# weixiaopassking/GS-LIVM

Measured on AMD Instinct MI355X. Metric: rasterizer fwd+bwd Mpixels/s @1920x1080, 2000000 Gaussians (ms_per_step = ms/frame), higher is better.
Workload: dtype f32; 1 GPU; C3: 2000000 Gaussians, 1920x1080, SH degree 0, 1 view per GPU per step, fwd+bwd + Adam step; view_threads=1, camera=one fixed view, near_entries=0, parallelism=view-parallel x1, adam_in_step=True, optimizer=one-kernel tail: activation chain rule + Adam + next activations (HIP), loss=seeded

## Files before the change

gs-livm_amd/__init__.py:

```python
from . import multiview, synthetic
from ._capi import (GsrError, LIB_PATH, NumRendered, emit_guard_trips, last_num_rendered, lib, mailbox_slow_path_last, mark_visible,
                    set_binning_capacity_hint, speculation_stats, set_near_far, set_near_far_thread, set_reference_rects_thread, async_outcomes_pending, set_near_far_hints, last_near_far, set_far_speculation, last_far_skipped, profile_enable, profile_read,
                    pose_gradient, rasterize_backward, rasterize_forward, reference_rects, set_reference_rects, state_views)
from .loss import (DeltaDepthLoss, ExposureLoss, LidarDepthLoss, PhotometricLoss, SimilarityLoss, delta_depth_loss, delta_pose,
                   apply_exposure, exposure_photometric_loss, identity_exposure, lidar_depth_image, lidar_depth_loss,
                   photometric_loss, raster_K, reference_window_1d, similarity_loss,
                   world_to_camera)
from .covis import (KeyframeVisibility, covisibility, iou, observation_count, overlap_coefficient,
                    visibility_pack, visibility_remap)
from .metrics import depth_to_u8, evaluate_keyframes, image_metrics, psnr, side_by_side, to_u8
from .model import FusedActivations, FusedAdam, GaussianParameters, GrowableAdam, GrowableGaussians, VoxelIndex, prune_rows
from . import ply
from .rasterizer import (GaussianRasterizationSettings, GaussianRasterizer,
                         rasterize_gaussians)
from .render_utils import Camera, get_projection_matrix, render, render_full, se3_exp



def torch_ops():
    import importlib.util
    import os
    import torch
    lib()
    path = os.path.join(os.path.dirname(os.path.abspath(__file__)), "_gsraster_torch.so")
    if not os.path.exists(path):
        raise RuntimeError("_gsraster_torch.so not built: run `python gs-livm_amd/build.py`")
    spec = importlib.util.spec_from_file_location("_gsraster_torch", path)
    mod = importlib.util.module_from_spec(spec)
    spec.loader.exec_module(mod)
    return mod


__all__ = ["KeyframeVisibility", "visibility_pack", "covisibility", "observation_count", "visibility_remap", "iou", "overlap_coefficient", "ExposureLoss", "exposure_photometric_loss", "apply_exposure", "identity_exposure", "LidarDepthLoss", "lidar_depth_image", "lidar_depth_loss", "raster_K", "world_to_camera", "prune_rows", "image_metrics", "psnr", "to_u8", "side_by_side", "depth_to_u8", "evaluate_keyframes", "DeltaDepthLoss", "delta_depth_loss", "delta_pose", "SimilarityLoss", "similarity_loss", "VoxelIndex", "PhotometricLoss", "photometric_loss", "reference_window_1d", "FusedActivations", "FusedAdam", "GaussianParameters", "GrowableAdam", "GrowableGaussians", "ply", "GaussianRasterizationSettings", "GaussianRasterizer", "rasterize_gaussians", "Camera", "render", "render_full", "se3_exp", "pose_gradient", "get_projection_matrix", "rasterize_forward",
           "rasterize_backward", "mark_visible", "state_views", "set_reference_rects", "reference_rects", "last_num_rendered", "set_binning_capacity_hint", "speculation_stats", "emit_guard_trips", "mailbox_slow_path_last", "set_near_far", "set_near_far_thread", "set_reference_rects_thread", "async_outcomes_pending", "set_near_far_hints", "last_near_far", "set_far_speculation", "last_far_skipped", "NumRendered", "lib", "torch_ops", "synthetic", "multiview", "GsrError", "LIB_PATH"]
```

gs-livm_amd/_capi.py:

```python
import ctypes as C
import os

import torch

_HERE = os.path.dirname(os.path.abspath(__file__))
LIB_PATH = os.environ.get("GSR_LIB", os.path.join(_HERE, "libgsraster_hip.so"))

ALLOC_FN = C.CFUNCTYPE(C.c_void_p, C.c_void_p, C.c_size_t)


class GeometryView(C.Structure):
    _fields_ = [(n, C.c_void_p) for n in
                ("depths", "radii", "splats", "cov3D", "tiles_touched", "point_offsets", "clamped", "depth_order",
                 "num_rendered", "gpack")]


class BinningView(C.Structure):
    _fields_ = [("point_list", C.c_void_p)]


class ImageView(C.Structure):
    _fields_ = [(n, C.c_void_p) for n in ("ranges", "final_T", "n_contrib", "quad_last", "ranges_far")]


class MailboxEvent(C.Structure):
    _fields_ = [("count", C.c_uint), ("ticket_expected", C.c_uint32), ("ticket_seen_before_query", C.c_uint32),
                ("elapsed_us", C.c_double), ("ticket_seen_after_query", C.c_uint32), ("first_query_result", C.c_int),
                ("visible_at_query", C.c_int), ("queries", C.c_uint), ("longest_query_us", C.c_double),
                ("longest_poll_gap_us", C.c_double)]


class NumRendered(int):

    def __new__(cls, exact, key):
        obj = super().__new__(cls, exact)
        obj.key = int(key)
        return obj


def _key(R):
    return int(getattr(R, "key", R))


_lib = None

EXPORTS = ("gsr_forward", "gsr_backward", "gsr_backward_depth", "gsr_mark_visible", "gsr_geometry_bytes", "gsr_image_bytes",
           "gsr_binning_bytes", "gsr_geometry_view_of", "gsr_binning_view_of", "gsr_image_view_of",
           "gsr_higher_msb", "gsr_last_error", "gsr_abi_version", "gsr_kernel_count", "gsr_kernel_name",
           "gsr_profile_enable", "gsr_profile_enable_only", "gsr_profile_read", "gsr_mailbox_slow_path_hits", "gsr_activate", "gsr_activate_backward", "gsr_adam_step",
           "gsr_photometric_loss", "gsr_photometric_loss_workspace", "gsr_init_gaussians", "gsr_ply_row_floats",
           "gsr_pack_ply_rows", "gsr_model_step", "gsr_set_reference_rects", "gsr_reference_rects",
           "gsr_last_num_rendered", "gsr_set_binning_capacity_hint", "gsr_speculative_forwards",
           "gsr_speculation_overflows", "gsr_emit_guard_trips", "gsr_mailbox_slow_path_last", "gsr_set_near_far", "gsr_near_far",
           "gsr_last_near_far", "gsr_set_near_far_hints", "gsr_near_far_forwards", "gsr_set_far_speculation",
           "gsr_last_far_skipped", "gsr_far_skips", "gsr_far_skip_misses", "gsr_async_far_frames",
           "gsr_near_budget_scale", "gsr_near_budget_feedback", "gsr_near_far_pause", "gsr_set_near_far_thread",
           "gsr_set_reference_rects_thread", "gsr_async_outcomes_pending", "gsr_async_outcomes_lost",
           "gsr_frame_note_misses", "gsr_similarity_loss", "gsr_similarity_loss_workspace",
           "gsr_delta_depth_loss", "gsr_delta_depth_loss_workspace", "gsr_image_metrics",
           "gsr_image_metrics_workspace", "gsr_pack_image_u8", "gsr_pack_depth_u8", "gsr_prune_workspace",
           "gsr_prune_mark", "gsr_prune_compact", "gsr_lidar_depth_image", "gsr_lidar_depth_loss",
           "gsr_lidar_depth_loss_workspace", "gsr_density_accumulate", "gsr_densify_workspace", "gsr_densify_mark",
           "gsr_densify_apply", "gsr_pose_gradient", "gsr_pose_gradient_workspace", "gsr_exposure_loss",
           "gsr_exposure_loss_workspace", "gsr_apply_exposure", "gsr_visibility_words", "gsr_visibility_pack",
           "gsr_covisibility", "gsr_observation_count", "gsr_visibility_remap")


def lib():
    global _lib
    if _lib is not None:
        return _lib
    if not os.path.exists(LIB_PATH):
        raise RuntimeError(
            "libgsraster_hip.so not built: run `python gs-livm_amd/build.py` (needs hipcc). "
            "gs_livm_amd has no CPU fallback.")
    L = C.CDLL(LIB_PATH)
    vp, ci, cf, sz = C.c_void_p, C.c_int, C.c_float, C.c_size_t
    L.gsr_forward.restype = ci
    L.gsr_forward.argtypes = [ALLOC_FN, vp, ALLOC_FN, vp, ALLOC_FN, vp, ci, ci, ci, vp, ci, ci, vp, vp, vp, vp, vp, cf,
                              vp, vp, vp, vp, vp, cf, cf, ci, vp, vp, vp, vp, ci, vp]
    L.gsr_backward.restype = ci
    L.gsr_backward.argtypes = [ci, ci, ci, ci, vp, ci, ci, vp, vp, vp, vp, cf, vp, vp, vp, vp, vp, cf, cf, vp, vp, vp,
                               vp, vp, vp, vp, vp, vp, vp, vp, vp, vp, vp, vp, ci, vp]
    L.gsr_backward_depth.restype = ci
    L.gsr_backward_depth.argtypes = L.gsr_backward.argtypes[:25] + [vp] + L.gsr_backward.argtypes[25:34] + [vp, ci, vp]
    L.gsr_mark_visible.restype = ci
    L.gsr_mark_visible.argtypes = [ci, vp, vp, vp, vp, vp]
    L.gsr_pose_gradient_workspace.restype = sz
    L.gsr_pose_gradient_workspace.argtypes = [ci]
    L.gsr_pose_gradient.restype = ci
    L.gsr_pose_gradient.argtypes = [ci, ci, ci, vp, vp, cf, vp, vp, vp, vp, cf, cf, vp, vp, vp, vp, vp, vp, vp, sz, vp]
    for n in ("gsr_geometry_bytes", "gsr_binning_bytes"):
        getattr(L, n).restype = sz
        getattr(L, n).argtypes = [ci]
    L.gsr_image_bytes.restype = sz
    L.gsr_image_bytes.argtypes = [ci, ci]
    L.gsr_geometry_view_of.argtypes = [vp, ci, C.POINTER(GeometryView)]
    L.gsr_binning_view_of.argtypes = [vp, ci, C.POINTER(BinningView)]
    L.gsr_image_view_of.argtypes = [vp, ci, ci, C.POINTER(ImageView)]
    L.gsr_higher_msb.restype = C.c_uint32
    L.gsr_higher_msb.argtypes = [C.c_uint32]
    L.gsr_last_error.restype = C.c_char_p
    L.gsr_abi_version.restype = ci
    L.gsr_kernel_count.restype = ci
    L.gsr_kernel_name.restype = C.c_char_p
    L.gsr_kernel_name.argtypes = [ci]
    L.gsr_profile_enable.argtypes = [ci]
    L.gsr_profile_enable_only.argtypes = [C.POINTER(ci), ci]
    L.gsr_set_reference_rects.restype = ci
    L.gsr_set_reference_rects.argtypes = [ci]
    L.gsr_reference_rects.restype = ci
    L.gsr_reference_rects.argtypes = []
    L.gsr_last_num_rendered.restype = ci
    L.gsr_last_num_rendered.argtypes = []
    L.gsr_set_binning_capacity_hint.restype = C.c_longlong
    L.gsr_set_binning_capacity_hint.argtypes = [C.c_longlong]
    for n in ("gsr_speculative_forwards", "gsr_speculation_overflows", "gsr_emit_guard_trips"):
        getattr(L, n).restype = C.c_ulonglong
        getattr(L, n).argtypes = []
    L.gsr_set_near_far.restype = ci
    L.gsr_set_near_far.argtypes = [ci]
    L.gsr_near_far.restype = ci
    L.gsr_near_far.argtypes = []
    L.gsr_last_near_far.restype = ci
    L.gsr_last_near_far.argtypes = [C.POINTER(C.c_uint), C.POINTER(C.c_uint)]
    L.gsr_set_near_far_hints.restype = None
    L.gsr_set_near_far_hints.argtypes = [C.c_longlong, C.c_longlong]
    L.gsr_near_far_forwards.restype = C.c_ulonglong
    L.gsr_near_far_forwards.argtypes = []
    L.gsr_set_far_speculation.restype = ci
    L.gsr_set_far_speculation.argtypes = [ci]
    L.gsr_last_far_skipped.restype = ci
    L.gsr_last_far_skipped.argtypes = []
    L.gsr_near_budget_scale.restype = C.c_uint
    L.gsr_near_budget_scale.argtypes = []
    L.gsr_near_budget_feedback.restype = C.c_uint
    L.gsr_near_budget_feedback.argtypes = [C.c_uint, C.c_uint, C.c_uint]
    L.gsr_near_far_pause.restype = ci
    L.gsr_near_far_pause.argtypes = [ci]
    for n in ("gsr_far_skips", "gsr_far_skip_misses", "gsr_async_far_frames", "gsr_async_outcomes_lost",
              "gsr_frame_note_misses", "gsr_similarity_loss", "gsr_similarity_loss_workspace"):
        getattr(L, n).restype = C.c_ulonglong
        getattr(L, n).argtypes = []
    for n in ("gsr_set_near_far_thread", "gsr_set_reference_rects_thread"):
        getattr(L, n).restype = ci
        getattr(L, n).argtypes = [ci]
    L.gsr_async_outcomes_pending.restype = ci
    L.gsr_async_outcomes_pending.argtypes = []
    L.gsr_mailbox_slow_path_last.restype = ci
    L.gsr_mailbox_slow_path_last.argtypes = [C.POINTER(MailboxEvent)]
    L.gsr_mailbox_slow_path_hits.restype = C.c_ulonglong
    L.gsr_mailbox_slow_path_hits.argtypes = []
    L.gsr_profile_read.restype = ci
    L.gsr_profile_read.argtypes = [ci, C.POINTER(C.c_double), C.POINTER(ci)]
    L.gsr_activate.restype = ci
    L.gsr_activate.argtypes = [ci, ci] + [vp] * 9 + [vp]
    L.gsr_activate_backward.restype = ci
    L.gsr_activate_backward.argtypes = [ci, ci] + [vp] * 12 + [vp]
    L.gsr_photometric_loss_workspace.restype = sz
    L.gsr_photometric_loss_workspace.argtypes = [ci, ci, ci]
    L.gsr_photometric_loss.restype = ci
    L.gsr_photometric_loss.argtypes = [ci, ci, ci, vp, vp, C.POINTER(cf), cf, vp, vp, vp, sz, vp]
    L.gsr_exposure_loss_workspace.restype = sz
    L.gsr_exposure_loss_workspace.argtypes = [ci, ci, ci]
    L.gsr_exposure_loss.restype = ci
    L.gsr_exposure_loss.argtypes = [ci, ci, ci, vp, vp, vp, C.POINTER(cf), cf, vp, vp, vp, vp, sz, vp]
    L.gsr_apply_exposure.restype = ci
    L.gsr_apply_exposure.argtypes = [ci, ci, ci, vp, vp, vp, vp]
    L.gsr_similarity_loss_workspace.restype = sz
    L.gsr_similarity_loss_workspace.argtypes = [ci, ci]
    L.gsr_similarity_loss.restype = ci
    L.gsr_similarity_loss.argtypes = [ci, ci, ci, vp, vp, vp, vp, cf, vp, vp, vp, ci, vp, sz, vp]
    L.gsr_delta_depth_loss_workspace.restype = sz
    L.gsr_delta_depth_loss_workspace.argtypes = [ci, ci]
    L.gsr_delta_depth_loss.restype = ci
    L.gsr_delta_depth_loss.argtypes = [ci, ci, vp, vp, vp, vp, C.POINTER(cf), C.POINTER(cf), C.POINTER(cf), cf, vp, vp,
                                       vp, vp, vp, sz, vp]
    L.gsr_lidar_depth_image.restype = ci
    L.gsr_lidar_depth_image.argtypes = [ci, vp, C.POINTER(cf), C.POINTER(cf), ci, ci, cf, cf, vp, vp, vp]
    L.gsr_lidar_depth_loss_workspace.restype = sz
    L.gsr_lidar_depth_loss_workspace.argtypes = [ci, ci]
    L.gsr_lidar_depth_loss.restype = ci
    L.gsr_lidar_depth_loss.argtypes = [ci, ci, vp, vp, vp, cf, cf, vp, vp, vp, vp, sz, vp]
    L.gsr_image_metrics_workspace.restype = sz
    L.gsr_image_metrics_workspace.argtypes = [ci, ci, ci]
    L.gsr_image_metrics.restype = ci
    L.gsr_image_metrics.argtypes = [ci, ci, ci, vp, vp, C.POINTER(cf), vp, vp, vp, sz, vp]
    L.gsr_pack_image_u8.restype = ci
    L.gsr_pack_image_u8.argtypes = [ci, ci, vp, ci, vp, sz, vp]
    L.gsr_pack_depth_u8.restype = ci
    L.gsr_pack_depth_u8.argtypes = [ci, ci, vp, cf, vp, sz, vp]
    L.gsr_prune_workspace.restype = sz
    L.gsr_prune_workspace.argtypes = [ci]
    L.gsr_prune_mark.restype = ci
    L.gsr_prune_mark.argtypes = [ci, vp, vp, vp, vp, vp, cf, cf, ci, vp, vp, vp, vp, sz, vp]
    L.gsr_prune_compact.restype = ci
    L.gsr_prune_compact.argtypes = [ci, ci, C.POINTER(vp), C.POINTER(vp), C.POINTER(ci), vp, vp, vp]
    L.gsr_density_accumulate.restype = ci
    L.gsr_density_accumulate.argtypes = [ci, vp, vp, vp, vp]
    L.gsr_densify_workspace.restype = sz
    L.gsr_densify_workspace.argtypes = [ci]
    L.gsr_densify_mark.restype = ci
    L.gsr_densify_mark.argtypes = [ci, vp, vp, cf, cf, ci, vp, vp, vp, vp, sz, vp]
    L.gsr_densify_apply.restype = ci
    L.gsr_densify_apply.argtypes = [ci, ci, ci, vp, vp, C.c_ulonglong] + [vp] * 6 + [C.POINTER(vp), C.POINTER(vp), vp, vp]
    ll = C.c_longlong
    L.gsr_visibility_words.restype = sz
    L.gsr_visibility_words.argtypes = [ci]
    L.gsr_visibility_pack.restype = ci
    L.gsr_visibility_pack.argtypes = [ci, vp, vp, vp, ci, vp]
    L.gsr_covisibility.restype = ci
    L.gsr_covisibility.argtypes = [ci, vp, ll, ci, vp, ll, ci, vp, vp, vp, vp]
    L.gsr_observation_count.restype = ci
    L.gsr_observation_count.argtypes = [ci, vp, ll, ci, ci, ci, vp, vp, vp]
    L.gsr_visibility_remap.restype = ci
    L.gsr_visibility_remap.argtypes = [ci, vp, ll, ci, vp, vp, vp, ll, ci, vp]
    L.gsr_init_gaussians.restype = ci
    L.gsr_init_gaussians.argtypes = [ci, ci, vp, vp, vp, cf] + [vp] * 6 + [vp]
    L.gsr_ply_row_floats.restype = sz
    L.gsr_ply_row_floats.argtypes = [ci]
    L.gsr_pack_ply_rows.restype = ci
    L.gsr_pack_ply_rows.argtypes = [ci, ci] + [vp] * 7 + [vp]
    L.gsr_model_step.restype = ci
    L.gsr_model_step.argtypes = [ci, ci, C.POINTER(vp), C.POINTER(vp), C.POINTER(vp)] + [vp] * 9 + \
        [C.POINTER(cf), C.c_double, C.c_double, C.c_double, ci, vp]
    L.gsr_adam_step.restype = ci
    L.gsr_adam_step.argtypes = [ci, C.POINTER(vp), C.POINTER(vp), C.POINTER(vp), C.POINTER(vp), C.POINTER(sz),
                                C.POINTER(cf), C.c_double, C.c_double, C.c_double, ci, ci, vp]
    _lib = L
    return L

# ... 118 lines not shown
        out = out + (dL_dconic,)
    return out + (dL_ddepths,) if grad_depth is not None else out


def pose_gradient(means3D, radii, scales, rotations, scale_modifier, cov3D_precomp, viewmatrix, projmatrix, tan_fovx,
                  tan_fovy, image_height, image_width, dL_dmeans2D, dL_dconic, dL_dmeans3D, dL_ddepths=None,
                  workspace=None):
    dev = means3D.device
    P = int(means3D.size(0))
    L = lib()
    need = int(L.gsr_pose_gradient_workspace(P))
    if workspace is None:
        workspace = torch.empty(need, dtype=torch.uint8, device=dev)
    out = torch.empty(6, dtype=torch.float32, device=dev)
    rotations = _rot16(rotations)
    _check(L.gsr_pose_gradient(P, int(image_width), int(image_height), _ptr(means3D), _ptr(scales),
                               float(scale_modifier), _ptr(rotations), _ptr(cov3D_precomp), _ptr(viewmatrix),
                               _ptr(projmatrix), float(tan_fovx), float(tan_fovy), _ptr(radii), _ptr(dL_dmeans2D),
                               _ptr(dL_dconic), _ptr(dL_ddepths), _ptr(dL_dmeans3D), _ptr(out), _ptr(workspace),
                               workspace.numel(), _stream()))
    return out


def last_num_rendered():
    return int(lib().gsr_last_num_rendered())


def set_binning_capacity_hint(capacity):
    return int(lib().gsr_set_binning_capacity_hint(-1 if capacity is None else int(capacity)))


def speculation_stats():
    L = lib()
    return dict(speculative_forwards=int(L.gsr_speculative_forwards()), overflows=int(L.gsr_speculation_overflows()),
                near_far_forwards=int(L.gsr_near_far_forwards()), far_skips=int(L.gsr_far_skips()),
                far_skip_misses=int(L.gsr_far_skip_misses()), async_far_frames=int(L.gsr_async_far_frames()),
                async_outcomes_lost=int(L.gsr_async_outcomes_lost()), frame_note_misses=int(L.gsr_frame_note_misses()),
                near_budget_scale_q8=int(L.gsr_near_budget_scale()),
                mailbox_slow_path_hits=int(L.gsr_mailbox_slow_path_hits()))


def emit_guard_trips():
    return int(lib().gsr_emit_guard_trips())


def mailbox_slow_path_last():
    ev = MailboxEvent()
    _check(lib().gsr_mailbox_slow_path_last(C.byref(ev)))
    return {n: getattr(ev, n) for n, _ in MailboxEvent._fields_}


def set_near_far(on):
    return bool(lib().gsr_set_near_far(int(bool(on))))


def set_near_far_thread(mode):
    prev = int(lib().gsr_set_near_far_thread(-1 if mode is None else int(bool(mode))))
    return None if prev < 0 else bool(prev)


def async_outcomes_pending():
    return int(lib().gsr_async_outcomes_pending())


def set_near_far_hints(near_entries_per_tile=None, far_capacity=None):
    lib().gsr_set_near_far_hints(-1 if near_entries_per_tile is None else int(near_entries_per_tile),
                                 -1 if far_capacity is None else int(far_capacity))


def set_far_speculation(mode):
    return int(lib().gsr_set_far_speculation(-1 if mode is None else int(bool(mode))))


def last_far_skipped():
    return bool(lib().gsr_last_far_skipped())


def last_near_far():
    a, b = C.c_uint(0), C.c_uint(0)
    split = bool(lib().gsr_last_near_far(C.byref(a), C.byref(b)))
    return split, int(a.value), int(b.value)


def set_reference_rects(on):
    return bool(lib().gsr_set_reference_rects(int(bool(on))))


def set_reference_rects_thread(mode):
    prev = int(lib().gsr_set_reference_rects_thread(-1 if mode is None else int(bool(mode))))
    return None if prev < 0 else bool(prev)


def reference_rects():
    return bool(lib().gsr_reference_rects())


def mark_visible(means3D, viewmatrix, projmatrix):
    P = int(means3D.size(0))
    present = torch.zeros((P,), dtype=torch.bool, device=means3D.device)
    if P:
        _check(lib().gsr_mark_visible(P, _ptr(means3D), _ptr(viewmatrix), _ptr(projmatrix),
                                      C.c_void_p(present.data_ptr()), _stream()))
    return present


def _sub(blob, ptr, count, dtype):
    if not ptr or count == 0:
        return None
    off = int(ptr) - blob.data_ptr()
    nbytes = count * torch.empty((), dtype=dtype).element_size()
    return blob[off:off + nbytes].view(dtype)


def state_views(geomBuffer, binningBuffer, imageBuffer, P, R, W, H):
    L = lib()
    gv, bv, iv = GeometryView(), BinningView(), ImageView()
    T = ((W + 15) // 16) * ((H + 15) // 16)
    out = {}
    if P:
        _check(L.gsr_geometry_view_of(_ptr(geomBuffer), P, C.byref(gv)))
        splats = _sub(geomBuffer, gv.splats, P * 12, torch.float32).view(P, 12)
        gpack = _sub(geomBuffer, gv.gpack, P * 2, torch.int32).view(P, 2)
        out.update(depths=splats[:, 9],
                   radii=_sub(geomBuffer, gv.radii, P, torch.int32),
                   splats=splats,
                   cov3D=_sub(geomBuffer, gv.cov3D, P * 6, torch.float32).view(P, 6),
                   tiles_touched=gpack[:, 0],
                   point_offsets=_sub(geomBuffer, gv.point_offsets, P, torch.int32),
                   clamped=_sub(geomBuffer, gv.clamped, P, torch.uint8),
                   depth_order=_sub(geomBuffer, gv.depth_order, P, torch.int32))
        _check(L.gsr_image_view_of(_ptr(imageBuffer), W, H, C.byref(iv)))
        out.update(ranges=_sub(imageBuffer, iv.ranges, T * 2, torch.int32).view(T, 2),
                   final_T=_sub(imageBuffer, iv.final_T, W * H, torch.float32).view(H, W),
                   n_contrib=_sub(imageBuffer, iv.n_contrib, W * H, torch.int32).view(H, W),
                   quad_last=_sub(imageBuffer, iv.quad_last, T * 4, torch.int32).view(T, 4))
        counters = _sub(geomBuffer, gv.num_rendered, 16, torch.int32).cpu().tolist()
        split = counters[12] == 1
        exact = counters[6] + counters[8] if split else counters[0]
        out.update(num_rendered=exact, near_far=split, counters=counters)
        key = _key(R)
        if exact:
            _check(L.gsr_binning_view_of(_ptr(binningBuffer), key, C.byref(bv)))
            raw = _sub(binningBuffer, bv.point_list, key, torch.int32)
            ra = out["ranges"].long()
            rb = _sub(imageBuffer, iv.ranges_far, T * 2, torch.int32).view(T, 2).long()
            seg_start = torch.stack([ra[:, 0], rb[:, 0]], 1).reshape(-1)
            seg_len = torch.stack([ra[:, 1] - ra[:, 0], rb[:, 1] - rb[:, 0]], 1).reshape(-1)
            total = int(seg_len.sum())
            excl = torch.cumsum(seg_len, 0) - seg_len
            idx = torch.repeat_interleave(seg_start - excl, seg_len) + torch.arange(total, device=ra.device)
            point_list = raw[idx]
            ln = seg_len.view(T, 2).sum(1)
            ends = torch.cumsum(ln, 0)
            ranges = torch.stack([ends - ln, ends], 1)
            ranges[ln == 0] = 0
            out.update(ranges_near=out["ranges"], ranges_far=rb.int(), ranges=ranges.int())
            tile_ids = torch.repeat_interleave(torch.arange(T, device=ra.device), ln)
            dbits = out["depths"].view(torch.int32)[point_list.long()].long() & 0xFFFFFFFF
            out.update(tile_ids=tile_ids, point_list=point_list, keys=(tile_ids.long() << 32) | dbits)
    return out


def profile_enable(on=True, only=None):
    L = lib()
    if on and only is not None:
        names = [L.gsr_kernel_name(i).decode() for i in range(L.gsr_kernel_count())]
# ... 340 lines not shown
```

gs-livm_amd/csrc/api.hip:

```cpp
#include "../../include/gsraster.h"

#include <algorithm>
#include <atomic>
#include <mutex>
#include <cstdarg>
#include <cstdio>
#include <cstdlib>
#include <cstring>
#include <chrono>
#include <cmath>
#include <unordered_map>
#include <vector>

#include "gsr_api.hpp"
#include "gsr_internal.hpp"

using namespace gsr;

static thread_local char g_err[512] = "";

namespace gsr {
int fail(int code, const char* fmt, ...) {
  va_list ap;
  va_start(ap, fmt);
  vsnprintf(g_err, sizeof(g_err), fmt, ap);
  va_end(ap);
  return code;
}
void clear_error() { g_err[0] = 0; }
}

#define STAGE(expr)                                                                               \
  do {                                                                                            \
    HIP_TRY(expr);                                                                                \
    if (debug) HIP_TRY(hipStreamSynchronize(stream));                                             \
  } while (0)

namespace gsr {
const Env& env() {
  static const Env e = [] {
    const auto set = [](const char* v) { return v != nullptr; };
    const auto not_zero = [](const char* v) { return !(v && v[0] == '0'); };
    Env x;
    const char* v = getenv("GSR_REFERENCE_RECTS");
    x.reference_rects = v && v[0] && v[0] != '0';
    x.near_far = not_zero(getenv("GSR_NEAR_FAR"));
    x.async_far = not_zero(getenv("GSR_ASYNC_FAR"));
    x.sync_forward = set(getenv("GSR_SYNC_FORWARD"));
    v = getenv("GSR_NEAR_ENTRIES");
    x.near_entries = v ? atol(v) : 320;
    v = getenv("GSR_NEAR_FAR_MIN_RATIO_Q2");
    x.near_far_min_ratio_q2 = v ? strtoull(v, nullptr, 10) : 12ull;
    x.full_depth_sort = set(getenv("GSR_FULL_DEPTH_SORT"));
    x.depth_hist_pass = set(getenv("GSR_DEPTH_HIST_PASS"));
    v = getenv("GSR_PRE_HIST_MIN_P");
    x.pre_hist_min_p = v ? std::max(0L, atol(v)) : -1;
    x.ranges_from_keys = set(getenv("GSR_RANGES_FROM_KEYS"));
    x.tile_sort_lsd = set(getenv("GSR_TILE_SORT_LSD"));
    x.sort_two_level_scan = set(getenv("GSR_SORT_TWO_LEVEL_SCAN"));
    x.sort_ballot_rank = set(getenv("GSR_SORT_BALLOT_RANK"));
    x.blend_backward_quads = set(getenv("GSR_BLEND_BACKWARD_QUADS"));
    x.blend_backward_tiles = set(getenv("GSR_BLEND_BACKWARD_TILES"));
    x.bwd_image_order = set(getenv("GSR_BWD_IMAGE_ORDER"));
    x.gbwd_all = set(getenv("GSR_GBWD_ALL"));
    x.host_trace = set(getenv("GSR_HOST_TRACE"));
    return x;
  }();
  return e;
}
}

namespace gsr {
std::atomic<bool> g_prof_on{false};
std::atomic<unsigned long long> g_prof_mask{~0ull};
thread_local bool t_prof_suppress = false;
static std::mutex g_ev_mu;
static std::vector<hipEvent_t> g_ev;
static std::vector<int> g_ev_id;
static size_t g_ev_used = 0;
void prof_begin(int id, hipStream_t s) {
  g_ev_mu.lock();
  if (g_ev_used == g_ev_id.size()) {
    hipEvent_t a, b;
    if (hipEventCreate(&a) != hipSuccess || hipEventCreate(&b) != hipSuccess) {
      g_prof_on = false;
      g_ev_id.push_back(-1);
      g_ev.push_back(nullptr); g_ev.push_back(nullptr);
      return;
    }
    g_ev.push_back(a); g_ev.push_back(b); g_ev_id.push_back(id);
  }
  g_ev_id[g_ev_used] = id;
  if (g_ev[2 * g_ev_used]) (void)hipEventRecord(g_ev[2 * g_ev_used], s);
}
void prof_end(hipStream_t s) {
  if (g_ev_used < g_ev_id.size() && g_ev[2 * g_ev_used + 1]) {
    (void)hipEventRecord(g_ev[2 * g_ev_used + 1], s);
    g_ev_used++;
  }
  g_ev_mu.unlock();
}
}
static const char* const kKernelNames[K_COUNT] = {
    "k_preprocess", "k_point_offsets", "k_scan_offsets", "k_emit",
    "k_sort_hist", "k_sort_scan_chunks", "k_sort_scan_top", "k_sort_scatter", "k_tile_ranges", "k_blend_forward",
    "k_blend_backward", "k_compact_touched", "k_gather_records", "k_gaussian_backward", "k_mark_visible", "k_sort_hist[depth]",
    "k_sort_scan_chunks[depth]", "k_sort_scan_top[depth]", "k_sort_scatter[depth]", "k_activate",
    "k_activate_backward", "k_adam", "k_loss_forward", "k_loss_finalize", "k_loss_backward", "k_init_gaussians", "k_pack_ply_rows", "k_model_step", "k_tile_order", "k_live_sat", "k_compact_near",
    "k_simi_nearest", "k_simi_points", "k_simi_grads",
    "k_delta_project", "k_delta_sample", "k_delta_scatter", "k_delta_convert",
    "k_visibility",
    "k_lidar_clear", "k_lidar_splat", "k_lidar_convert", "k_lidar_loss_forward", "k_lidar_loss_finish",
    "k_lidar_loss_grads",
    "k_density_accumulate", "k_densify_mark", "k_densify_scan", "k_densify_rank", "k_densify_apply",
    "k_pose_partials", "k_pose_finish",
    "k_exposure_loss_forward", "k_exposure_loss_backward", "k_exposure_loss_finish", "k_apply_exposure",
    "k_metrics_forward", "k_metrics_finalize", "k_pack_image_u8", "k_pack_depth_u8",
    "k_prune_mark", "k_prune_scan", "k_prune_rank", "k_prune_compact"};
static_assert(K_COUNT <= 64, "g_prof_mask is one 64-bit word");

extern "C" {

int gsr_kernel_count(void) { return K_COUNT; }
const char* gsr_kernel_name(int id) { return (id >= 0 && id < K_COUNT) ? kKernelNames[id] : ""; }
int gsr_profile_enable(int on) {
  std::lock_guard<std::mutex> lk(g_ev_mu);
  if (on) g_ev_used = 0;
  g_prof_on = on != 0;
  g_prof_mask = ~0ull;
  return GSR_OK;
}
int gsr_profile_enable_only(const int* kernel_ids, int n) {
  if (!kernel_ids && n > 0) return fail(GSR_ERR_INVALID_ARGUMENT, "null kernel id list");
  unsigned long long m = 0;
  for (int i = 0; i < n; i++) {
    if (kernel_ids[i] < 0 || kernel_ids[i] >= K_COUNT) return fail(GSR_ERR_INVALID_ARGUMENT, "bad kernel id");
    m |= 1ull << kernel_ids[i];
  }
  std::lock_guard<std::mutex> lk(g_ev_mu);
  g_ev_used = 0;
  g_prof_mask = m;
  g_prof_on = true;
  return GSR_OK;
}
int gsr_profile_read(int max_ids, double* total_ms, int* launches) {
  const int n = max_ids < K_COUNT ? max_ids : (int)K_COUNT;
  std::lock_guard<std::mutex> lk(g_ev_mu);
// ... 958 lines not shown
  lazy_resolve(g_ctx);
  return (int)g_ctx.last_R;
}
int gsr_set_near_far(int on) { return near_far_flag().exchange(on != 0 ? 1 : 0); }
int gsr_set_near_far_thread(int mode) {
  const int prev = t_near_far;
  t_near_far = mode < 0 ? -1 : (mode ? 1 : 0);
  return prev;
}
int gsr_near_far(void) { return t_near_far >= 0 ? t_near_far : near_far_flag().load(); }
int gsr_last_near_far(unsigned* near_instances, unsigned* far_instances) {
  lazy_resolve(g_ctx);
  if (near_instances) *near_instances = g_ctx.last_near;
  if (far_instances) *far_instances = g_ctx.last_far;
  return g_ctx.last_was_near_far ? 1 : 0;
}
void gsr_set_near_far_hints(long long near_entries_per_tile, long long far_capacity) {
  g_ctx.near_entries_override = near_entries_per_tile < 0 ? -1 : near_entries_per_tile;
  g_ctx.far_hint_override = far_capacity < 0 ? -1 : (far_capacity > 0x7fffffffll ? 0x7fffffffll : far_capacity);
  if (far_capacity < 0)
    for (auto& v : g_ctx.views) v.have_far = false;
}
unsigned long long gsr_near_far_forwards(void) { return g_near_far_forwards.load(); }
int gsr_set_far_speculation(int mode) {
  const int prev = g_ctx.far_skip_override;
  g_ctx.far_skip_override = mode < 0 ? -1 : (mode ? 1 : 0);
  if (mode < 0)
    for (auto& v : g_ctx.views) v.far_idle_streak = 0;
  return prev;
}
int gsr_last_far_skipped(void) {
  lazy_resolve(g_ctx);
  return g_ctx.last_far_skipped ? 1 : 0;
}
unsigned long long gsr_async_far_frames(void) { return g_async_frames.load(); }
unsigned gsr_near_budget_scale(void) {
  lazy_resolve(g_ctx);
  return g_ctx.views[g_ctx.cur].near_scale_q8;
}
unsigned gsr_near_budget_feedback(unsigned unfinished_quads, unsigned near_instances, unsigned far_instances) {
  budget_feedback(g_ctx, g_ctx.views[g_ctx.cur], unfinished_quads, near_instances, far_instances);
  return g_ctx.views[g_ctx.cur].near_scale_q8;
}
int gsr_near_far_pause(int frames) {
  const int prev = g_ctx.views[g_ctx.cur].split_pause;
  if (frames >= 0) g_ctx.views[g_ctx.cur].split_pause = frames;
  return prev;
}
unsigned long long gsr_far_skips(void) { return g_far_skips.load(); }
unsigned long long gsr_far_skip_misses(void) { return g_far_skip_misses.load(); }
long long gsr_set_binning_capacity_hint(long long capacity) {
  const long long prev = g_ctx.hint_override;
  g_ctx.hint_override = capacity < 0 ? -1 : (capacity > 0x7fffffffll ? 0x7fffffffll : capacity);
  if (capacity == 0)
    for (auto& v : g_ctx.views) v.recent.clear();
  return prev;
}
unsigned long long gsr_speculative_forwards(void) { return g_speculative_forwards.load(); }
unsigned long long gsr_speculation_overflows(void) { return g_speculation_overflows.load(); }
unsigned long long gsr_emit_guard_trips(void) { return emit_guard_trips(); }
int gsr_mailbox_slow_path_last(gsr_mailbox_event* out) {
  if (!out) return fail(GSR_ERR_INVALID_ARGUMENT, "null pointer");
  std::lock_guard<std::mutex> lk(g_slow_mu);
  *out = g_slow_last;
  return GSR_OK;
}

int gsr_set_reference_rects(int on) { return reference_rects_flag().exchange(on != 0 ? 1 : 0); }
int gsr_reference_rects(void) { return t_reference_rects >= 0 ? t_reference_rects : reference_rects_flag().load(); }
int gsr_set_reference_rects_thread(int mode) {
  const int prev = t_reference_rects;
  t_reference_rects = mode < 0 ? -1 : (mode ? 1 : 0);
  return prev;
}
unsigned long long gsr_frame_note_misses(void) { return g_note_misses.load(); }
unsigned long long gsr_async_outcomes_lost(void) { return g_async_outcomes_lost.load(); }
int gsr_async_outcomes_pending(void) {
  lazy_resolve(g_ctx);
  return g_ctx.pending_n;
}

unsigned long long gsr_mailbox_slow_path_hits(void) { return g_mailbox_slow_hits.load(); }

static int backward_impl(bool with_depth, int P, int D, int M, int R, const float* background, int width, int height,
                         const float* means3D, const float* shs, const float* colors_precomp, const float* scales,
                         float scale_modifier, const float* rotations, const float* cov3D_precomp,
                         const float* viewmatrix, const float* projmatrix, const float* campos, float tan_fovx,
                         float tan_fovy, const int* radii, char* geom_buffer, char* binning_buffer, char* image_buffer,
                         const float* dL_dpix, const float* dL_dacc, const float* dL_ddepth, float* dL_dmean2D,
                         float* dL_dconic, float* dL_dopacity, float* dL_dcolor, float* dL_dmean3D, float* dL_dcov3D,
                         float* dL_dsh, float* dL_dscale, float* dL_drot, float* dL_ddepths, int debug,
                         void* stream_) {
  hipStream_t stream = (hipStream_t)stream_;
  g_err[0] = 0;
  if (P < 0 || R < 0 || width <= 0 || height <= 0) return fail(GSR_ERR_INVALID_ARGUMENT, "bad P/R/width/height");
  if (P == 0) return GSR_OK;
  if (!geom_buffer || !binning_buffer || !image_buffer) return fail(GSR_ERR_INVALID_ARGUMENT, "null state blob");
  if (!means3D || !background || !viewmatrix || !projmatrix || !campos || !dL_dpix || !dL_dacc)
    return fail(GSR_ERR_INVALID_ARGUMENT, "null required input");
  if (!dL_dmean2D || !dL_dconic || !dL_dopacity || !dL_dcolor || !dL_dmean3D || (!dL_dcov3D && cov3D_precomp) ||
      !dL_dscale || !dL_drot || (M > 0 && !dL_dsh))
    return fail(GSR_ERR_INVALID_ARGUMENT, "null gradient output");
  if (with_depth && !dL_ddepth) return fail(GSR_ERR_INVALID_ARGUMENT, "null dL_ddepth");
  if (with_depth && !dL_ddepths) return fail(GSR_ERR_INVALID_ARGUMENT, "null dL_ddepths");
  if (!cov3D_precomp && (!scales || !rotations))
    return fail(GSR_ERR_INVALID_ARGUMENT, "provide scales+rotations or a precomputed 3D covariance");
  if (!colors_precomp && (D < 0 || D > 3 || M < (D + 1) * (D + 1) || M > 16))
    return fail(GSR_ERR_UNSUPPORTED, "SH degree %d with %d coefficients is not supported (D<=3, (D+1)^2<=M<=16)", D, M);
  if (!cov3D_precomp && misaligned16(rotations)) return fail_rotations(rotations);
  if (env().host_trace)
    fprintf(stderr, "[gsr] backward entered at %.1f us (process clock)\n",
            std::chrono::duration<double, std::micro>(std::chrono::steady_clock::now().time_since_epoch()).count());
  const FrameParams fp = make_params(P, D, M, width, height, tan_fovx, tan_fovy, scale_modifier);
  GeomState g = GeomState::carve(geom_buffer, (size_t)P);
  BinningState b = BinningState::carve(binning_buffer, (size_t)R);
  ImageState im = ImageState::carve(image_buffer, width, height);
  if (!radii) radii = g.radii;

  if (R > 0) {
    const unsigned notes = frame_notes(image_buffer);
    STAGE(launch_blend_backward(fp, g, b, im, background, dL_dpix, dL_dacc, dL_ddepth, (notes & NOTE_ORDER) != 0u,
                                stream));
    STAGE(launch_gather_records(fp, g, b, dL_dmean2D, dL_dconic, dL_dopacity, dL_dcolor, dL_ddepths,
                                (notes & NOTE_SPLIT) != 0u, stream));
  }
  STAGE(launch_gaussian_backward(fp, g, b, radii, means3D, scales, rotations, colors_precomp ? nullptr : shs,
                                 cov3D_precomp, viewmatrix, projmatrix, campos, colors_precomp != nullptr, dL_dmean2D,
                                 dL_dconic, dL_dopacity, dL_dcolor, dL_dmean3D, dL_dcov3D, dL_dsh, dL_dscale, dL_drot,
                                 dL_ddepths, stream));
  return GSR_OK;
}

int gsr_backward(int P, int D, int M, int R, const float* background, int width, int height, const float* means3D,
                 const float* shs, const float* colors_precomp, const float* scales, float scale_modifier,
                 const float* rotations, const float* cov3D_precomp, const float* viewmatrix,
                 const float* projmatrix, const float* campos, float tan_fovx, float tan_fovy, const int* radii,
                 char* geom_buffer, char* binning_buffer, char* image_buffer, const float* dL_dpix,
                 const float* dL_dacc, float* dL_dmean2D, float* dL_dconic, float* dL_dopacity, float* dL_dcolor,
                 float* dL_dmean3D, float* dL_dcov3D, float* dL_dsh, float* dL_dscale, float* dL_drot, int debug,
                 void* stream_) {
  return backward_impl(false, P, D, M, R, background, width, height, means3D, shs, colors_precomp, scales,
                       scale_modifier, rotations, cov3D_precomp, viewmatrix, projmatrix, campos, tan_fovx, tan_fovy, radii,
                       geom_buffer, binning_buffer, image_buffer, dL_dpix, dL_dacc, nullptr, dL_dmean2D, dL_dconic,
                       dL_dopacity, dL_dcolor, dL_dmean3D, dL_dcov3D, dL_dsh, dL_dscale, dL_drot, nullptr, debug, stream_);
}

int gsr_backward_depth(int P, int D, int M, int R, const float* background, int width, int height,
                       const float* means3D, const float* shs, const float* colors_precomp, const float* scales,
                       float scale_modifier, const float* rotations, const float* cov3D_precomp,
                       const float* viewmatrix, const float* projmatrix, const float* campos, float tan_fovx,
                       float tan_fovy, const int* radii, char* geom_buffer, char* binning_buffer, char* image_buffer,
                       const float* dL_dpix, const float* dL_dacc, const float* dL_ddepth, float* dL_dmean2D,
                       float* dL_dconic, float* dL_dopacity, float* dL_dcolor, float* dL_dmean3D, float* dL_dcov3D,
                       float* dL_dsh, float* dL_dscale, float* dL_drot, float* dL_ddepths, int debug, void* stream_) {
  return backward_impl(true, P, D, M, R, background, width, height, means3D, shs, colors_precomp, scales, scale_modifier,
                       rotations, cov3D_precomp, viewmatrix, projmatrix, campos, tan_fovx, tan_fovy, radii, geom_buffer,
                       binning_buffer, image_buffer, dL_dpix, dL_dacc, dL_ddepth, dL_dmean2D, dL_dconic, dL_dopacity,
                       dL_dcolor, dL_dmean3D, dL_dcov3D, dL_dsh, dL_dscale, dL_drot, dL_ddepths, debug, stream_);
}

size_t gsr_pose_gradient_workspace(int P) { return P < 0 ? 0 : pose_workspace_bytes(P); }

int gsr_pose_gradient(int P, int width, int height, const float* means3D, const float* scales, float scale_modifier,
                      const float* rotations, const float* cov3D_precomp, const float* viewmatrix,
                      const float* projmatrix, float tan_fovx, float tan_fovy, const int* radii,
                      const float* dL_dmean2D, const float* dL_dconic, const float* dL_ddepths,
                      const float* dL_dmean3D, float* dL_dpose, char* workspace, size_t workspace_bytes,
                      void* stream_) {
  g_err[0] = 0;
  if (P < 0) return fail(GSR_ERR_INVALID_ARGUMENT, "bad P (%d)", P);
  if (width <= 0 || height <= 0) return fail(GSR_ERR_INVALID_ARGUMENT, "bad width/height (%d x %d)", width, height);
  if (!(tan_fovx > 0.f) || !(tan_fovy > 0.f) || !std::isfinite(tan_fovx) || !std::isfinite(tan_fovy))
    return fail(GSR_ERR_INVALID_ARGUMENT, "tan_fovx / tan_fovy must be finite and positive");
  if (!dL_dpose) return fail(GSR_ERR_INVALID_ARGUMENT, "null dL_dpose");
  if (!workspace) return fail(GSR_ERR_INVALID_ARGUMENT, "null workspace");
  if (P > 0) {
    if (!means3D || !viewmatrix || !projmatrix || !radii) return fail(GSR_ERR_INVALID_ARGUMENT, "null required input");
    if (!dL_dmean2D || !dL_dconic || !dL_dmean3D) return fail(GSR_ERR_INVALID_ARGUMENT, "null gradient input");
    if (cov3D_precomp ? (scales || rotations) : (!scales || !rotations))
      return fail(GSR_ERR_INVALID_ARGUMENT, "provide either scales+rotations or a precomputed 3D covariance");
    if (!cov3D_precomp && misaligned16(rotations)) return fail_rotations(rotations);
  }
  if (int e = check_workspace(workspace_bytes, pose_workspace_bytes(P))) return e;
  const FrameParams fp = make_params(P, 0, 0, width, height, tan_fovx, tan_fovy, scale_modifier);
  HIP_TRY(launch_pose_gradient(fp, radii, means3D, scales, rotations, cov3D_precomp, viewmatrix, projmatrix, dL_dmean2D,
                               dL_dconic, dL_ddepths, dL_dmean3D, dL_dpose, workspace, (hipStream_t)stream_));
  return GSR_OK;
}

int gsr_mark_visible(int P, const float* means3D, const float* viewmatrix, const float* projmatrix,
                     unsigned char* present, void* stream_) {
  (void)projmatrix;
  g_err[0] = 0;
  if (P < 0) return fail(GSR_ERR_INVALID_ARGUMENT, "bad P");
  if (P == 0) return GSR_OK;
  if (!means3D || !viewmatrix || !present) return fail(GSR_ERR_INVALID_ARGUMENT, "null pointer");
  HIP_TRY(launch_mark_visible(P, means3D, viewmatrix, present, (hipStream_t)stream_));
  return GSR_OK;
}

int gsr_geometry_view_of(char* geom_buffer, int P, gsr_geometry_view* out) {
  if (!geom_buffer || !out || P < 0) return fail(GSR_ERR_INVALID_ARGUMENT, "bad argument");
  GeomState g = GeomState::carve(geom_buffer, (size_t)P);
  out->depths = nullptr;
  out->radii = g.radii;
  out->splats = reinterpret_cast<const float*>(g.splats);
  out->cov3D = g.cov3D;
  out->tiles_touched = nullptr;
  out->gpack = reinterpret_cast<const uint32_t*>(g.gpack);
  out->point_offsets = g.point_offsets;
  out->clamped = g.clamped;
  out->depth_order = g.order;
// ... 24 lines not shown
```

gs-livm_amd/csrc/gsr_internal.hpp:

```cpp
#pragma once
#include <hip/hip_runtime.h>
#include <atomic>
#include <stddef.h>
#include <stdint.h>

namespace gsr {

constexpr int TILE = 16;
constexpr int SPLAT_F4 = 3;
constexpr int GRAD_F4 = 3;
constexpr int PRE_BLOCK = 256;
constexpr int SORT_TILE = 4096;
constexpr int TSORT_TILE = 4096;
constexpr int TSORT_WAVES = 4;
constexpr int EMIT_CHUNK = 2048;
constexpr int SORT_CHUNK = 64;
constexpr size_t ALIGN = 256;

inline size_t align_up(size_t v) { return (v + ALIGN - 1) & ~(ALIGN - 1); }

struct Carver {
  char* base;
  size_t off = 0;
  explicit Carver(char* b) : base(b) {}
// ... 138 lines not shown
struct BinningState {
  uint32_t* point_list;
  uint32_t* tkeysA;
  uint32_t* tkeysB;
  uint32_t* ivalsB;
  SortScratch tsort;
  float4* grad_inst;
  uint8_t* inst_flag;
  uint32_t* chunk_first;
  uint32_t* chunk_firstB;
  static BinningState carve(char* blob, size_t R, size_t* bytes = nullptr) {
    Carver c(blob);
    BinningState b;
    b.point_list = c.take<uint32_t>(R);
    size_t mark = align_up(c.off);
    b.tkeysA = c.take<uint32_t>(R);
    b.tkeysB = c.take<uint32_t>(R);
    b.ivalsB = c.take<uint32_t>(R);
    SortScratch::carve(c, R, b.tsort);
    size_t sort_end = c.off;
    Carver g(blob);
    g.off = mark;
    b.grad_inst = g.take<float4>(R * GRAD_F4);
    c.off = sort_end > g.off ? sort_end : g.off;
    b.inst_flag = c.take<uint8_t>(R);
    b.chunk_first = c.take<uint32_t>(R / EMIT_CHUNK + 2);
    b.chunk_firstB = c.take<uint32_t>(R / EMIT_CHUNK + 2);
    if (bytes) *bytes = align_up(c.off) + ALIGN;
    return b;
  }
};

struct Count {
  const uint32_t* dev;
  int cap;
  const uint32_t* gate = nullptr;
  uint32_t gate_open = 0;
  bool bounded = false;
  __device__ __forceinline__ bool closed() const { return gate && __builtin_nontemporal_load(gate) != gate_open; }
  __device__ __forceinline__ int get() const {
    if (!dev) return cap;
    const uint32_t v = __builtin_nontemporal_load(dev);
    return v < (uint32_t)cap ? (int)v : cap;
  }
};

constexpr int GATED_GRID_MAX = 1024;
template <typename F>
__device__ __forceinline__ void for_each_unit(const int nunits, F&& f) {
  for (int unit = blockIdx.x; unit < nunits; unit += gridDim.x) {
    f(unit);
    __syncthreads();
  }
}
__host__ __device__ inline int units_of(int n, int per) { return (int)(((long long)n + per - 1) / per); }
inline int chain_grid(const Count& c, int per) {
  const int u = units_of(c.cap, per);
  return (c.gate || c.bounded) && u > GATED_GRID_MAX ? GATED_GRID_MAX : u;
}
struct FrameParams {
  int P, D, M, W, H, gx, gy;
  float tan_fovx, tan_fovy, focal_x, focal_y, scale_modifier;
  int ref_rects;
};

struct Env {
  bool reference_rects;
  bool near_far;
  bool async_far;
  bool sync_forward;
  long near_entries;
  unsigned long long near_far_min_ratio_q2;
  bool full_depth_sort;
  bool depth_hist_pass;
  long pre_hist_min_p;
  bool ranges_from_keys;
  bool tile_sort_lsd;
  bool sort_two_level_scan;
  bool sort_ballot_rank;
  bool blend_backward_quads;
  bool blend_backward_tiles;
  bool bwd_image_order;
  bool gbwd_all;
  bool host_trace;
};
const Env& env();

bool preprocess_counts_depth_digits(const FrameParams& fp, const float* shs, const float* colors_precomp);
hipError_t launch_preprocess(const FrameParams& fp, const float* means3D, const float* scales, const float* rotations,
                             const float* opacities, const float* shs, const float* cov3D_precomp,
                             const float* colors_precomp, const float* view, const float* proj, const float* campos,
                             GeomState g, int* radii_out, bool write_cov3D, unsigned long long* done_word,
                             unsigned long long* publish, uint32_t ticket, uint32_t* ghist_acc, uint32_t* ghist_clear,
                             hipStream_t s);
hipError_t launch_point_offsets(const FrameParams& fp, GeomState g, hipStream_t s);
hipError_t launch_scan_offsets(const FrameParams& fp, GeomState g, Count R, uint32_t* chunk_first, uint2* ranges,
                               uint2* rangesB, uint32_t* counts0, uint32_t near_budget,
                               unsigned long long* publish_near, uint32_t ticket, const uint32_t* top_hist,
                               const uint32_t* order, bool order_is_near_list, hipStream_t s);
hipError_t launch_compact_near(const FrameParams& fp, GeomState g, const uint32_t* top_hist, uint32_t near_budget,
                               uint32_t* keys_out, uint32_t* vals_out, uint32_t* n_out, uint32_t* ghist_near,
                               unsigned long long* publish, uint32_t ticket, hipStream_t s);
hipError_t launch_clear_words(Count gate, uint32_t* words, size_t n, hipStream_t s);
hipError_t launch_scan_offsets_far(const FrameParams& fp, GeomState g, Count capB, uint32_t slot_base, const uint32_t* sat,
                                   uint32_t* chunk_firstB, uint32_t* counts0, unsigned long long* publish,
                                   uint32_t ticket, hipStream_t s);
unsigned long long emit_guard_trips();
hipError_t launch_emit(const FrameParams& fp, const uint4* sdesc, Count R, uint32_t* chunk_first, uint32_t* tkeys_out,
                       uint32_t* ivals_out, uint8_t* inst_flag, uint32_t* counts0, uint32_t digit_shift0,
                       uint32_t digit_mask0, bool key16, bool store_pairs, hipStream_t s);
struct EmitFusion {
  FrameParams fp;
  const uint4* sdesc;
  Count R;
  const uint32_t* chunk_first;
};
hipError_t launch_emit_scatter(const EmitFusion& ef, uint16_t* keys_out, uint32_t* vals_out, int shift0, int nbits0,
                               const uint32_t* counts, const uint32_t* chunk_base, const uint32_t* digit_total,
                               bool arank, hipStream_t s);
constexpr int TILE_SORT_BUCKETS_MAX = 16 << 20;
bool tile_sort_buckets(int tile_bits, bool key16, int capacity);
struct BucketPass {
  uint2* ranges;
  int tiles;
  uint32_t list_base;
};
hipError_t launch_gather_records(const FrameParams& fp, GeomState g, BinningState b, float* dL_dmean2D,
                                 float* dL_dconic, float* dL_dopacity, float* dL_dcolor, float* dL_ddepths,
                                 bool split_frame, hipStream_t s);
hipError_t launch_sort_pairs(uint32_t* keysA, uint32_t* valsA, uint32_t* keysB, uint32_t* valsB, SortScratch sc,
                             Count n, int end_bit, bool start_in_A, bool is_depth_sort, bool key16,
                             bool first_hist_done, const EmitFusion* fused_first_pass, uint32_t* key_count,
                             hipStream_t s, const BucketPass* buckets = nullptr);
hipError_t launch_depth_sort(uint32_t* keysA, uint32_t* valsA, uint32_t* keysB, uint32_t* valsB, DepthSortScratch sc,
                             Count n, const uint32_t* ghist, bool vals_are_positions, hipStream_t s);
hipError_t launch_ranges_from_counts(uint2* ranges, int T, uint32_t list_base, Count gate, hipStream_t s);
hipError_t launch_verify_sorted_lists(const uint2* ranges, int T, const uint32_t* point_list, const float4* splats,
                                      uint32_t* violations, hipStream_t s);
hipError_t launch_tile_ranges(const uint32_t* tile_ids, Count R, uint2* ranges, bool key16, uint32_t list_base, hipStream_t s);
struct AsyncWords {
  uint32_t* decide = nullptr;
  uint32_t* go = nullptr;
  uint32_t* gate_dev = nullptr;
  uint32_t seq = 0;
};
hipError_t launch_blend_forward(const FrameParams& fp, GeomState g, BinningState b, ImageState im, const float* bg,
                                float* out_color, float* out_depth, float* out_acc, int phase,
                                unsigned long long* done_word, unsigned long long* publish, uint32_t ticket,
                                AsyncWords aw, Count gate, hipStream_t s);
hipError_t launch_live_sat(const FrameParams& fp, ImageState im, uint32_t* total_live, Count gate, hipStream_t s);
hipError_t launch_release_go(Count gate, uint32_t* go, uint32_t seq, hipStream_t s);
hipError_t launch_decide_far(const uint32_t* live_quads, AsyncWords aw, hipStream_t s);
hipError_t launch_tile_order(const FrameParams& fp, ImageState im, hipStream_t s);
hipError_t launch_blend_backward(const FrameParams& fp, GeomState g, BinningState b, ImageState im, const float* bg,
                                 const float* dL_dpix, const float* dL_dacc, const float* dL_ddepth, bool have_tile_order,
                                 hipStream_t s);
hipError_t launch_gaussian_backward(const FrameParams& fp, GeomState g, BinningState b, const int* radii,
                                    const float* means3D, const float* scales, const float* rotations,
                                    const float* shs, const float* cov3D_precomp, const float* view, const float* proj,
                                    const float* campos, bool colors_precomp, float* dL_dmean2D, float* dL_dconic,
                                    float* dL_dopacity, float* dL_dcolor, float* dL_dmean3D, float* dL_dcov3D,
                                    float* dL_dsh, float* dL_dscale, float* dL_drot, float* dL_ddepths,
                                    hipStream_t s);
hipError_t launch_mark_visible(int P, const float* means3D, const float* view, unsigned char* present, hipStream_t s);
size_t pose_workspace_bytes(int P);
hipError_t launch_pose_gradient(const FrameParams& fp, const int* radii, const float* means3D, const float* scales,
                                const float* rotations, const float* cov3D_precomp, const float* view,
                                const float* proj, const float* dL_dmean2D, const float* dL_dconic,
                                const float* dL_ddepths, const float* dL_dmean3D, float* dL_dpose, char* workspace,
                                hipStream_t s);

inline int sort_passes(int end_bit) { return (end_bit + 7) / 8; }
inline int sort_digit_bits(int end_bit) { const int p = sort_passes(end_bit); return (end_bit + p - 1) / p; }

enum KernelId {
  K_PREPROCESS = 0, K_POINT_OFFSETS, K_SCAN_OFFSETS, K_EMIT, K_SORT_HIST,
  K_SORT_SCAN_CHUNKS, K_SORT_SCAN_TOP, K_SORT_SCATTER, K_TILE_RANGES, K_BLEND_FWD, K_BLEND_BWD, K_COMPACT_TOUCHED,
  K_GATHER_RECORDS, K_GAUSSIAN_BWD, K_MARK_VISIBLE, K_DSORT_HIST, K_DSORT_SCAN_CHUNKS, K_DSORT_SCAN_TOP,
  K_DSORT_SCATTER, K_ACTIVATE, K_ACTIVATE_BWD, K_ADAM, K_LOSS_FWD, K_LOSS_FINALIZE, K_LOSS_BWD, K_INIT_GAUSSIANS, K_PACK_PLY, K_MODEL_STEP, K_TILE_ORDER, K_LIVE_SAT, K_COMPACT_NEAR,
  K_SIMI_NEAREST, K_SIMI_POINTS, K_SIMI_GRADS,
  K_DELTA_PROJECT, K_DELTA_SAMPLE, K_DELTA_SCATTER, K_DELTA_CONVERT,
  K_VISIBILITY,
  K_LIDAR_CLEAR, K_LIDAR_SPLAT, K_LIDAR_CONVERT, K_LIDAR_LOSS_FWD, K_LIDAR_LOSS_FINISH, K_LIDAR_LOSS_GRADS,
  K_DENSITY_ACCUMULATE, K_DENSIFY_MARK, K_DENSIFY_SCAN, K_DENSIFY_RANK, K_DENSIFY_APPLY,
  K_POSE_PARTIALS, K_POSE_FINISH,
  K_EXPOSURE_LOSS_FWD, K_EXPOSURE_LOSS_BWD, K_EXPOSURE_LOSS_FINISH, K_APPLY_EXPOSURE,
  K_METRICS_FWD, K_METRICS_FINALIZE, K_PACK_IMAGE_U8, K_PACK_DEPTH_U8,
  K_PRUNE_MARK, K_PRUNE_SCAN, K_PRUNE_RANK, K_PRUNE_COMPACT, K_COUNT
};
void prof_begin(int id, hipStream_t s);
void prof_end(hipStream_t s);
extern std::atomic<bool> g_prof_on;
extern std::atomic<unsigned long long> g_prof_mask;
extern thread_local bool t_prof_suppress;
struct ProfScope {
  hipStream_t s;
  bool on;
  ProfScope(int id, hipStream_t st)
      : s(st), on(!t_prof_suppress && g_prof_on.load(std::memory_order_relaxed) &&
                  ((g_prof_mask.load(std::memory_order_relaxed) >> id) & 1ull)) {
    if (on) prof_begin(id, s);
  }
  ~ProfScope() { if (on) prof_end(s); }
};

__device__ __forceinline__ float sigmoidf_(float x) { return 1.0f / (1.0f + expf(-x)); }

__device__ __forceinline__ float ln_upper(float x) {
  const uint32_t b = __float_as_uint(x);
  const int e = (int)(b >> 23) - 127;
  const float m = __uint_as_float((b & 0x007FFFFFu) | 0x3F800000u);
  const float t = (m - 1.0f) / (m + 1.0f);
  const float t2 = t * t;
  const float s = t * (2.0f + t2 * (0.6666667f + t2 * 0.4f));
  return (float)e * 0.6931472f + s + 3e-4f;
}

__device__ __forceinline__ float footprint_tau(float op) { return ln_upper(255.0f * op) * 1.01f + 0.02f; }

__host__ __device__ inline void tile_rect(float px, float py, int radius, int gx, int gy, int& x0, int& y0, int& x1,
                                          int& y1) {
  const float r = (float)radius;
  int a = (int)((px - r) / 16.0f), b = (int)((py - r) / 16.0f);
  int c = (int)((((px + r) + 16.0f) - 1.0f) / 16.0f), d = (int)((((py + r) + 16.0f) - 1.0f) / 16.0f);
  a = a < 0 ? 0 : a; b = b < 0 ? 0 : b; c = c < 0 ? 0 : c; d = d < 0 ? 0 : d;
  x0 = a > gx ? gx : a; y0 = b > gy ? gy : b; x1 = c > gx ? gx : c; y1 = d > gy ? gy : d;
}

}
```

gs-livm_amd/csrc/preprocess.hip:

```cpp

#include "gsr_internal.hpp"
#include "sort_core.hpp"

namespace gsr {

__device__ __forceinline__ float fmin_(float a, float b) { return fminf(a, b); }
__device__ __forceinline__ float fmax_(float a, float b) { return fmaxf(a, b); }

__device__ __forceinline__ float ndc_to_pix(float v, int S) {
  return (float)((((double)v + 1.0) * (double)S - 1.0) * 0.5);
}

__device__ __forceinline__ uint32_t wave_sum_u32(uint32_t v) {
#pragma unroll
  for (int o = 32; o > 0; o >>= 1) v += __shfl_xor(v, o, 64);
  return v;
}

__device__ __forceinline__ unsigned long long wave_sum_u64(unsigned long long v) {
#pragma unroll
  for (int o = 32; o > 0; o >>= 1) v += __shfl_xor(v, o, 64);
  return v;
}

// ... 53 lines not shown
  e.T00 = V[0] * J00 + V[2] * J02;
  e.T01 = V[4] * J00 + V[6] * J02;
  e.T02 = V[8] * J00 + V[10] * J02;
  e.T10 = V[1] * J11 + V[2] * J12;
  e.T11 = V[5] * J11 + V[6] * J12;
  e.T12 = V[9] * J11 + V[10] * J12;
  const float S00 = c6[0], S01 = c6[1], S02 = c6[2], S11 = c6[3], S12 = c6[4], S22 = c6[5];
  const float A00 = e.T00 * S00 + e.T01 * S01 + e.T02 * S02;
  const float A10 = e.T00 * S01 + e.T01 * S11 + e.T02 * S12;
  const float A20 = e.T00 * S02 + e.T01 * S12 + e.T02 * S22;
  const float A01 = e.T10 * S00 + e.T11 * S01 + e.T12 * S02;
  const float A11 = e.T10 * S01 + e.T11 * S11 + e.T12 * S12;
  const float A21 = e.T10 * S02 + e.T11 * S12 + e.T12 * S22;
  e.cxx = A00 * e.T00 + A10 * e.T01 + A20 * e.T02;
  e.cxy = A01 * e.T00 + A11 * e.T01 + A21 * e.T02;
  e.cyy = A01 * e.T10 + A11 * e.T11 + A21 * e.T12;
  return e;
}

__device__ __forceinline__ int sh_row_stride(int C) { return C | 1; }

__device__ __forceinline__ void rows_to_lds(float* lds, const float* __restrict__ src, const int nrows, const int C) {
  const int n = nrows * C, S = sh_row_stride(C);
  if ((C & 3) == 0 && (reinterpret_cast<uintptr_t>(src) & 15u) == 0) {
    const int C4 = C >> 2, n4 = n >> 2;
    const int dr = PRE_BLOCK / C4, dc = PRE_BLOCK - dr * C4;
    int r = (int)threadIdx.x / C4, c4 = (int)threadIdx.x - r * C4;
    for (int j = threadIdx.x; j < n4; j += PRE_BLOCK) {
      const float4 v = reinterpret_cast<const float4*>(src)[j];
      float* d = lds + r * S + 4 * c4;
      d[0] = v.x; d[1] = v.y; d[2] = v.z; d[3] = v.w;
      r += dr; c4 += dc;
      if (c4 >= C4) { c4 -= C4; r++; }
    }
  } else {
    const int dr = PRE_BLOCK / C, dc = PRE_BLOCK - dr * C;
    int r = (int)threadIdx.x / C, c = (int)threadIdx.x - r * C;
    for (int e = threadIdx.x; e < n; e += PRE_BLOCK) {
      lds[r * S + c] = src[e];
      r += dr; c += dc;
      if (c >= C) { c -= C; r++; }
    }
  }
}

__device__ __forceinline__ void lds_to_rows(float* __restrict__ dst, const float* lds, const int nrows, const int C) {
  const int n = nrows * C, S = sh_row_stride(C);
  if ((C & 3) == 0 && (reinterpret_cast<uintptr_t>(dst) & 15u) == 0) {
    const int C4 = C >> 2, n4 = n >> 2;
    const int dr = PRE_BLOCK / C4, dc = PRE_BLOCK - dr * C4;
    int r = (int)threadIdx.x / C4, c4 = (int)threadIdx.x - r * C4;
    for (int j = threadIdx.x; j < n4; j += PRE_BLOCK) {
      const float* d = lds + r * S + 4 * c4;
      reinterpret_cast<float4*>(dst)[j] = make_float4(d[0], d[1], d[2], d[3]);
      r += dr; c4 += dc;
      if (c4 >= C4) { c4 -= C4; r++; }
    }
  } else {
    const int dr = PRE_BLOCK / C, dc = PRE_BLOCK - dr * C;
    int r = (int)threadIdx.x / C, c = (int)threadIdx.x - r * C;
    for (int e = threadIdx.x; e < n; e += PRE_BLOCK) {
      dst[e] = lds[r * S + c];
      r += dr; c += dc;
      if (c >= C) { c -= C; r++; }
    }
  }
}

__device__ __forceinline__ void listed_rows_to_lds(float* lds, const float* __restrict__ src, const uint32_t* list,
                                                   const int nlist, const int C) {
  const int S = sh_row_stride(C);
  if ((C & 3) == 0 && (reinterpret_cast<uintptr_t>(src) & 15u) == 0) {
    const int C4 = C >> 2;
    for (int k = threadIdx.x; k < nlist * C4; k += PRE_BLOCK) {
      const int r = (int)list[k / C4], c4 = k % C4;
      const float4 v = reinterpret_cast<const float4*>(src + (size_t)r * C)[c4];
      float* d = lds + r * S + 4 * c4;
      d[0] = v.x; d[1] = v.y; d[2] = v.z; d[3] = v.w;
    }
  } else {
    for (int k = threadIdx.x; k < nlist * C; k += PRE_BLOCK) {
      const int r = (int)list[k / C], c = k % C;
      lds[r * S + c] = src[(size_t)r * C + c];
    }
  }
}

static inline size_t sh_stage_bytes(int M) {
  if (M <= 1) return 0;
  const size_t b = (size_t)PRE_BLOCK * (size_t)((3 * M) | 1) * sizeof(float);
  return b <= 64 * 1024 ? b : 0;
}

template <bool STAGED, bool PLAIN = false, bool PIN = PLAIN, int ROWK = 0>
__global__ __launch_bounds__(PRE_BLOCK) void k_preprocess(
    const FrameParams fp, const float* __restrict__ means3D, const float* __restrict__ scales,
    const float* __restrict__ rotations, const float* __restrict__ opacities, const float* __restrict__ shs,
    const float* __restrict__ cov3D_precomp, const float* __restrict__ colors_precomp,
    const float* __restrict__ V, const float* __restrict__ Pm, const float* __restrict__ campos, GeomState g,
    int* __restrict__ radii_out, const bool write_cov3D, unsigned long long* __restrict__ done_word,
    unsigned long long* __restrict__ publish,
    const uint32_t ticket, uint32_t* __restrict__ ghist_acc, uint32_t* __restrict__ ghist_clear) {
  if (blockIdx.x == 0 && threadIdx.x == 0) { g.total[2] = 0u; g.total[11] = 0u; }
  float Vc[16], Pc[16];
#pragma unroll
  for (int k = 0; k < 16; k++) { Vc[k] = V[k]; Pc[k] = Pm[k]; }
  const float cam0 = campos[0], cam1 = campos[1], cam2 = campos[2];
  extern __shared__ float sh_rows[];
  __shared__ uint32_t dhist[5][256];
  __shared__ float4 s_rec[PRE_BLOCK / 64][64 * SPLAT_F4];
  if (ghist_acc) {
#pragma unroll
    for (int k = 0; k < 5; k++) dhist[k][threadIdx.x] = 0u;
    if (blockIdx.x == 0)
#pragma unroll
      for (int k = 0; k < 5; k++) ghist_clear[k * 256 + threadIdx.x] = 0u;
    __syncthreads();
  }
  struct In { float mx, my, mz, s0, s1, s2, op, dc0, dc1, dc2; float4 q; };
  const bool dc_direct = PLAIN || (!STAGED && shs && !colors_precomp);
  const int D = PLAIN ? 0 : fp.D;
  auto fetch = [&](const int i_) {
    In v;
    const int i = i_ < fp.P ? i_ : fp.P - 1;
    v.s0 = v.s1 = v.s2 = v.dc0 = v.dc1 = v.dc2 = 0.f;
    v.q = make_float4(0.f, 0.f, 0.f, 0.f);
    v.mx = means3D[3 * i]; v.my = means3D[3 * i + 1]; v.mz = means3D[3 * i + 2];
    if (PIN || scales) { v.s0 = scales[3 * i]; v.s1 = scales[3 * i + 1]; v.s2 = scales[3 * i + 2]; }
    if (PIN || !cov3D_precomp) v.q = reinterpret_cast<const float4*>(rotations)[i];
    v.op = opacities[i];
    if (dc_direct) {
      const float* r = shs + (size_t)i * fp.M * 3;
      v.dc0 = r[0]; v.dc1 = r[1]; v.dc2 = r[2];
    }
    return v;
  };
  uint32_t tiles_wg = 0;
  const int nblk = (fp.P + PRE_BLOCK - 1) / PRE_BLOCK;
  auto work = [&](const In& in, const int blk, auto&& before_stores) {
  const int idx_raw = blk * PRE_BLOCK + threadIdx.x;
  const bool dup = idx_raw >= fp.P;
  const int idx = dup ? fp.P - 1 : idx_raw;
  if (STAGED && !(ROWK > 0 && (blk + 1) * PRE_BLOCK <= fp.P)) {
    const int row0 = blk * PRE_BLOCK;
    if (blk != (int)blockIdx.x) __syncthreads();
    if (row0 < fp.P) rows_to_lds(sh_rows, shs + (size_t)row0 * fp.M * 3, min(PRE_BLOCK, fp.P - row0), fp.M * 3);
    __syncthreads();
  }
  uint32_t tiles = 0, rect_packed = 0, dkey = 0xFFFFFFFFu;
  int radius = 0;
  float4 rec0 = make_float4(0.f, 0.f, 0.f, 0.f), rec1 = rec0, rec2 = rec0;
  uint8_t clamp_out = 0;
  {
    const float mx = in.mx, my = in.my, mz = in.mz;
    const float pvz = Vc[2] * mx + Vc[6] * my + Vc[10] * mz + Vc[14];
    bool alive = !(pvz <= 0.2f);
    float s0 = 0, s1 = 0, s2 = 0;
    if (alive && (PIN || scales)) {
      s0 = fp.scale_modifier * in.s0;
      s1 = fp.scale_modifier * in.s1;
      s2 = fp.scale_modifier * in.s2;
      alive = !(s0 > 0.3f || s1 > 0.3f || s2 > 0.3f);
    }
    if (alive) {
      const float ph0 = Pc[0] * mx + Pc[4] * my + Pc[8] * mz + Pc[12];
      const float ph1 = Pc[1] * mx + Pc[5] * my + Pc[9] * mz + Pc[13];
// ... 1038 lines not shown
          t.v9 = acc;
        }
        const float4 ra = g.splats[(size_t)id * SPLAT_F4 + 0];
        const float4 rb = g.splats[(size_t)id * SPLAT_F4 + 1];
        gather_finish(t, id, lane, ra.z, ra.w, rb.x, rb.y, ddelx_dx, ddely_dy, dL_dmean2D, dL_dconic, dL_dopacity, dL_dcolor,
                      dL_ddepths);
      }
      __syncthreads();
    }
    __syncthreads();
  }
}

__device__ __forceinline__ void geometric_backward(const float mx, const float my, const float mz,
                                                   const FrameParams& fp, const float* c6,
                                                   const float* __restrict__ V, const float* __restrict__ Pm,
                                                   const float gmx, const float gmy, const float gca,
                                                   const float gcb, const float gcc, float* __restrict__ dL_dcov3D_row,
                                                   float* dcov, float& dm0, float& dm1, float& dm2) {
  const Ewa e = ewa_project(mx, my, mz, fp, c6, V);
  const float limx = 1.3f * fp.tan_fovx, limy = 1.3f * fp.tan_fovy;
  const float xmul = (e.txtz < -limx || e.txtz > limx) ? 0.f : 1.f;
  const float ymul = (e.tytz < -limy || e.tytz > limy) ? 0.f : 1.f;
  const float a = e.cxx + 0.3f, b = e.cxy, c = e.cyy + 0.3f;
  const float denom = a * c - b * b;
  float dL_da = 0, dL_db = 0, dL_dc = 0;
  const float denom2inv = 1.0f / ((denom * denom) + 0.0000001f);
#pragma unroll
  for (int k = 0; k < 6; k++) dcov[k] = 0.f;
  if (denom2inv != 0) {
    dL_da = denom2inv * (-c * c * gca + 2 * b * c * gcb + (denom - a * c) * gcc);
    dL_dc = denom2inv * (-a * a * gcc + 2 * a * b * gcb + (denom - a * c) * gca);
    dL_db = denom2inv * 2 * (b * c * gca - (denom + 2 * b * b) * gcb + a * b * gcc);
    dcov[0] = (e.T00 * e.T00 * dL_da + e.T00 * e.T10 * dL_db + e.T10 * e.T10 * dL_dc);
    dcov[3] = (e.T01 * e.T01 * dL_da + e.T01 * e.T11 * dL_db + e.T11 * e.T11 * dL_dc);
    dcov[5] = (e.T02 * e.T02 * dL_da + e.T02 * e.T12 * dL_db + e.T12 * e.T12 * dL_dc);
    dcov[1] = 2 * e.T00 * e.T01 * dL_da + (e.T00 * e.T11 + e.T01 * e.T10) * dL_db + 2 * e.T10 * e.T11 * dL_dc;
    dcov[2] = 2 * e.T00 * e.T02 * dL_da + (e.T00 * e.T12 + e.T02 * e.T10) * dL_db + 2 * e.T10 * e.T12 * dL_dc;
    dcov[4] = 2 * e.T02 * e.T01 * dL_da + (e.T01 * e.T12 + e.T02 * e.T11) * dL_db + 2 * e.T11 * e.T12 * dL_dc;
  }
  if (dL_dcov3D_row) {
#pragma unroll
    for (int k = 0; k < 6; k++) dL_dcov3D_row[k] = dcov[k];
  }
  const float S00 = c6[0], S01 = c6[1], S02 = c6[2], S11 = c6[3], S12 = c6[4], S22 = c6[5];
  const float u0 = e.T00 * S00 + e.T01 * S01 + e.T02 * S02, u1 = e.T00 * S01 + e.T01 * S11 + e.T02 * S12,
              u2 = e.T00 * S02 + e.T01 * S12 + e.T02 * S22;
  const float v0 = e.T10 * S00 + e.T11 * S01 + e.T12 * S02, v1 = e.T10 * S01 + e.T11 * S11 + e.T12 * S12,
              v2 = e.T10 * S02 + e.T11 * S12 + e.T12 * S22;
  const float dT00 = 2 * u0 * dL_da + v0 * dL_db, dT01 = 2 * u1 * dL_da + v1 * dL_db, dT02 = 2 * u2 * dL_da + v2 * dL_db;
  const float dT10 = 2 * v0 * dL_dc + u0 * dL_db, dT11 = 2 * v1 * dL_dc + u1 * dL_db, dT12 = 2 * v2 * dL_dc + u2 * dL_db;
  const float dJ00 = V[0] * dT00 + V[4] * dT01 + V[8] * dT02;
  const float dJ02 = V[2] * dT00 + V[6] * dT01 + V[10] * dT02;
  const float dJ11 = V[1] * dT10 + V[5] * dT11 + V[9] * dT12;
  const float dJ12 = V[2] * dT10 + V[6] * dT11 + V[10] * dT12;
  const float tz = 1.f / e.tz, tz2 = tz * tz, tz3 = tz2 * tz;
  const float hx = fp.focal_x, hy = fp.focal_y;
  const float dtx = xmul * -hx * tz2 * dJ02;
  const float dty = ymul * -hy * tz2 * dJ12;
  const float dtz = -hx * tz2 * dJ00 - hy * tz2 * dJ11 + (2 * hx * e.tx) * tz3 * dJ02 + (2 * hy * e.ty) * tz3 * dJ12;
  dm0 = V[0] * dtx + V[1] * dty + V[2] * dtz;
  dm1 = V[4] * dtx + V[5] * dty + V[6] * dtz;
  dm2 = V[8] * dtx + V[9] * dty + V[10] * dtz;
  {
    const float mh3 = Pm[3] * mx + Pm[7] * my + Pm[11] * mz + Pm[15];
    const float m_w = 1.0f / (mh3 + 0.0000001f);
    const float mul1 = (Pm[0] * mx + Pm[4] * my + Pm[8] * mz + Pm[12]) * m_w * m_w;
    const float mul2 = (Pm[1] * mx + Pm[5] * my + Pm[9] * mz + Pm[13]) * m_w * m_w;
    dm0 += (Pm[0] * m_w - Pm[3] * mul1) * gmx + (Pm[1] * m_w - Pm[3] * mul2) * gmy;
    dm1 += (Pm[4] * m_w - Pm[7] * mul1) * gmx + (Pm[5] * m_w - Pm[7] * mul2) * gmy;
    dm2 += (Pm[8] * m_w - Pm[11] * mul1) * gmx + (Pm[9] * m_w - Pm[11] * mul2) * gmy;
  }
}

template <bool DEPTH>
__device__ __forceinline__ void gaussian_backward_one(
    const int idx, float* row,
    const FrameParams& fp, GeomState& g, const int* __restrict__ radii, const float* __restrict__ means3D, const float* __restrict__ scales,
    const float* __restrict__ rotations, const float* __restrict__ shs, const float* __restrict__ cov3D_precomp,
    const float* __restrict__ V, const float* __restrict__ Pm, const float* __restrict__ campos,
    const int colors_are_precomp, float* dL_dmean2D, float* dL_dconic, float* dL_dopacity, float* dL_dcolor,
    float* __restrict__ dL_dmean3D,
    float* __restrict__ dL_dcov3D, float* __restrict__ dL_dsh, float* __restrict__ dL_dscale,
    float* __restrict__ dL_drot, float* dL_ddepths, const bool skip_recordless) {
  const int rad_in = radii[idx];
  const uint8_t touched_in = g.touched[idx];
  const bool vis = rad_in > 0;
  const int M = fp.M;
  float* gs = row ? row : dL_dsh + (size_t)idx * fp.M * 3;
  if (idx == 0) g.total[2] = 0u;
  const bool was_touched = touched_in != 0;
  if (was_touched) g.touched[idx] = 0;
  const bool rec = vis && was_touched;
  if (!rec && (skip_recordless || !vis)) {
    dL_dmean2D[3 * idx] = 0.f; dL_dmean2D[3 * idx + 1] = 0.f; dL_dmean2D[3 * idx + 2] = 0.f;
    dL_dconic[4 * idx] = 0.f; dL_dconic[4 * idx + 1] = 0.f; dL_dconic[4 * idx + 2] = 0.f; dL_dconic[4 * idx + 3] = 0.f;
    dL_dopacity[idx] = 0.f;
    if constexpr (DEPTH) dL_ddepths[idx] = 0.f;
    dL_dcolor[3 * idx] = 0.f; dL_dcolor[3 * idx + 1] = 0.f; dL_dcolor[3 * idx + 2] = 0.f;
    dL_dmean3D[3 * idx] = 0.f; dL_dmean3D[3 * idx + 1] = 0.f; dL_dmean3D[3 * idx + 2] = 0.f;
    if (dL_dcov3D) {
#pragma unroll
      for (int k = 0; k < 6; k++) dL_dcov3D[6 * (size_t)idx + k] = 0.f;
    }
    for (int k = 0; k < 3 * M; k++) gs[k] = 0.f;
    dL_dscale[3 * idx] = 0.f; dL_dscale[3 * idx + 1] = 0.f; dL_dscale[3 * idx + 2] = 0.f;
    dL_drot[4 * idx] = 0.f; dL_drot[4 * idx + 1] = 0.f; dL_drot[4 * idx + 2] = 0.f; dL_drot[4 * idx + 3] = 0.f;
    return;
  }
  const float gcol0 = rec ? dL_dcolor[3 * idx] : 0.f, gcol1 = rec ? dL_dcolor[3 * idx + 1] : 0.f, gcol2 = rec ? dL_dcolor[3 * idx + 2] : 0.f;
  const float gmx = rec ? dL_dmean2D[3 * idx] : 0.f, gmy = rec ? dL_dmean2D[3 * idx + 1] : 0.f;
  const float gca = rec ? dL_dconic[4 * idx] : 0.f, gcb = rec ? dL_dconic[4 * idx + 1] : 0.f, gcc = rec ? dL_dconic[4 * idx + 3] : 0.f;
  float gz = 0.f;
  if constexpr (DEPTH) {
    if (rec) gz = dL_ddepths[idx];
    else dL_ddepths[idx] = 0.f;
  }
  if (!rec) {
    dL_dmean2D[3 * idx] = 0.f; dL_dmean2D[3 * idx + 1] = 0.f;
    dL_dconic[4 * idx] = 0.f; dL_dconic[4 * idx + 1] = 0.f; dL_dconic[4 * idx + 3] = 0.f;
    dL_dopacity[idx] = 0.f;
    dL_dcolor[3 * idx] = 0.f; dL_dcolor[3 * idx + 1] = 0.f; dL_dcolor[3 * idx + 2] = 0.f;
  }
  const float mx = means3D[3 * idx], my = means3D[3 * idx + 1], mz = means3D[3 * idx + 2];
  const uint8_t clamped_in = g.clamped[idx];
  float4 q_in = make_float4(0.f, 0.f, 0.f, 0.f);
  float sc_in[3] = {0.f, 0.f, 0.f};
  if (scales) {
    q_in = reinterpret_cast<const float4*>(rotations)[idx];
    sc_in[0] = scales[3 * idx]; sc_in[1] = scales[3 * idx + 1]; sc_in[2] = scales[3 * idx + 2];
  }
  float c6[6];
  if (cov3D_precomp) {
#pragma unroll
    for (int k = 0; k < 6; k++) c6[k] = cov3D_precomp[6 * (size_t)idx + k];
  } else {
    cov3d_from_scale_rot(fp.scale_modifier * sc_in[0], fp.scale_modifier * sc_in[1], fp.scale_modifier * sc_in[2], q_in, c6);
  }
  const float* sh = row ? row : shs + (size_t)idx * fp.M * 3;
  dL_dmean2D[3 * idx + 2] = 0.f;
  dL_dconic[4 * idx + 2] = 0.f;
  float dcov[6];
  float dm0, dm1, dm2;
  geometric_backward(mx, my, mz, fp, c6, V, Pm, gmx, gmy, gca, gcb, gcc,
                     dL_dcov3D ? dL_dcov3D + 6 * (size_t)idx : nullptr, dcov, dm0, dm1, dm2);
  if (shs && !colors_are_precomp) {
    const uint8_t cb = clamped_in;
    const float gr[3] = {(cb & 1) ? 0.f : gcol0, (cb & 2) ? 0.f : gcol1, (cb & 4) ? 0.f : gcol2};
    const float q0 = mx - campos[0], q1 = my - campos[1], q2 = mz - campos[2];
    const float len = sqrtf(q0 * q0 + q1 * q1 + q2 * q2);
    const float x = q0 / len, y = q1 / len, z = q2 / len;
    float ddx = 0, ddy = 0, ddz = 0;
    const int D = fp.D;
    const int used = (D + 1) * (D + 1);
#pragma unroll
    for (int ch = 0; ch < 3; ch++) {
      const float gch = gr[ch];
      float c_[16];
#pragma unroll
      for (int k = 1; k < 16; k++) c_[k] = k < used ? sh[3 * k + ch] : 0.f;
      float dx_ = 0, dy_ = 0, dz_ = 0;
      gs[ch] = SH0 * gch;
      if (D > 0) {
        gs[3 + ch] = (-SH1 * y) * gch;
        gs[6 + ch] = (SH1 * z) * gch;
        gs[9 + ch] = (-SH1 * x) * gch;
        dx_ = -SH1 * c_[3];
        dy_ = -SH1 * c_[1];
        dz_ = SH1 * c_[2];
        if (D > 1) {
          const float xx = x * x, yy = y * y, zz = z * z, xy = x * y, yz = y * z, xz = x * z;
          gs[12 + ch] = (SH2c[0] * xy) * gch;
          gs[15 + ch] = (SH2c[1] * yz) * gch;
          gs[18 + ch] = (SH2c[2] * (2.f * zz - xx - yy)) * gch;
          gs[21 + ch] = (SH2c[3] * xz) * gch;
          gs[24 + ch] = (SH2c[4] * (xx - yy)) * gch;
          dx_ += SH2c[0] * y * c_[4] + SH2c[2] * 2.f * -x * c_[6] + SH2c[3] * z * c_[7] +
// ... 12 lines not shown
            dx_ += (SH3c[0] * c_[9] * 3.f * 2.f * xy + SH3c[1] * c_[10] * yz +
                    SH3c[2] * c_[11] * -2.f * xy + SH3c[3] * c_[12] * -3.f * 2.f * xz +
                    SH3c[4] * c_[13] * (-3.f * xx + 4.f * zz - yy) + SH3c[5] * c_[14] * 2.f * xz +
                    SH3c[6] * c_[15] * 3.f * (xx - yy));
            dy_ += (SH3c[0] * c_[9] * 3.f * (xx - yy) + SH3c[1] * c_[10] * xz +
                    SH3c[2] * c_[11] * (-3.f * yy + 4.f * zz - xx) + SH3c[3] * c_[12] * -3.f * 2.f * yz +
                    SH3c[4] * c_[13] * -2.f * xy + SH3c[5] * c_[14] * -2.f * yz +
                    SH3c[6] * c_[15] * -3.f * 2.f * xy);
            dz_ += (SH3c[1] * c_[10] * xy + SH3c[2] * c_[11] * 4.f * 2.f * yz +
                    SH3c[3] * c_[12] * 3.f * (2.f * zz - xx - yy) + SH3c[4] * c_[13] * 4.f * 2.f * xz +
                    SH3c[5] * c_[14] * (xx - yy));
          }
        }
      }
      ddx += dx_ * gch;
      ddy += dy_ * gch;
      ddz += dz_ * gch;
    }
    for (int k = used * 3; k < M * 3; k++) gs[k] = 0.f;
    const float sum2 = q0 * q0 + q1 * q1 + q2 * q2;
    const float inv32 = 1.0f / sqrtf(sum2 * sum2 * sum2);
    dm0 += ((+sum2 - q0 * q0) * ddx - q1 * q0 * ddy - q2 * q0 * ddz) * inv32;
    dm1 += (-q0 * q1 * ddx + (sum2 - q1 * q1) * ddy - q2 * q1 * ddz) * inv32;
    dm2 += (-q0 * q2 * ddx - q1 * q2 * ddy + (sum2 - q2 * q2) * ddz) * inv32;
  } else {
    for (int k = 0; k < M * 3; k++) gs[k] = 0.f;
  }
  if constexpr (DEPTH) {
    dm0 += V[2] * gz; dm1 += V[6] * gz; dm2 += V[10] * gz;
  }
  dL_dmean3D[3 * idx] = dm0; dL_dmean3D[3 * idx + 1] = dm1; dL_dmean3D[3 * idx + 2] = dm2;
  if (scales) {
    const float4 q = q_in;
    const float r = q.x, x = q.y, y = q.z, z = q.w;
    const float s[3] = {fp.scale_modifier * sc_in[0], fp.scale_modifier * sc_in[1], fp.scale_modifier * sc_in[2]};
    float R[3][3];
    R[0][0] = 1.f - 2.f * (y * y + z * z); R[0][1] = 2.f * (x * y - r * z); R[0][2] = 2.f * (x * z + r * y);
    R[1][0] = 2.f * (x * y + r * z); R[1][1] = 1.f - 2.f * (x * x + z * z); R[1][2] = 2.f * (y * z - r * x);
    R[2][0] = 2.f * (x * z - r * y); R[2][1] = 2.f * (y * z + r * x); R[2][2] = 1.f - 2.f * (x * x + y * y);
    const float dS[3][3] = {{dcov[0], 0.5f * dcov[1], 0.5f * dcov[2]},
                            {0.5f * dcov[1], dcov[3], 0.5f * dcov[4]},
                            {0.5f * dcov[2], 0.5f * dcov[4], dcov[5]}};
    float dMt[3][3];
#pragma unroll
    for (int cc = 0; cc < 3; cc++)
#pragma unroll
      for (int rr = 0; rr < 3; rr++) {
        const float v = (2.0f * (s[rr] * R[0][rr])) * dS[cc][0] + (2.0f * (s[rr] * R[1][rr])) * dS[cc][1] +
                        (2.0f * (s[rr] * R[2][rr])) * dS[cc][2];
        dMt[rr][cc] = v;
      }
    float ds[3];
#pragma unroll
    for (int k = 0; k < 3; k++) ds[k] = R[0][k] * dMt[k][0] + R[1][k] * dMt[k][1] + R[2][k] * dMt[k][2];
    dL_dscale[3 * idx] = ds[0]; dL_dscale[3 * idx + 1] = ds[1]; dL_dscale[3 * idx + 2] = ds[2];
#pragma unroll
    for (int k = 0; k < 3; k++)
#pragma unroll
      for (int rr = 0; rr < 3; rr++) dMt[k][rr] *= s[k];
#define Dm(ci, ri) dMt[ci][ri]
    const float dq0 = 2 * z * (Dm(0, 1) - Dm(1, 0)) + 2 * y * (Dm(2, 0) - Dm(0, 2)) + 2 * x * (Dm(1, 2) - Dm(2, 1));
    const float dq1 = 2 * y * (Dm(1, 0) + Dm(0, 1)) + 2 * z * (Dm(2, 0) + Dm(0, 2)) + 2 * r * (Dm(1, 2) - Dm(2, 1)) -
                      4 * x * (Dm(2, 2) + Dm(1, 1));
    const float dq2 = 2 * x * (Dm(1, 0) + Dm(0, 1)) + 2 * r * (Dm(2, 0) - Dm(0, 2)) + 2 * z * (Dm(1, 2) + Dm(2, 1)) -
                      4 * y * (Dm(2, 2) + Dm(0, 0));
    const float dq3 = 2 * r * (Dm(0, 1) - Dm(1, 0)) + 2 * x * (Dm(2, 0) + Dm(0, 2)) + 2 * y * (Dm(1, 2) + Dm(2, 1)) -
                      4 * z * (Dm(1, 1) + Dm(0, 0));
#undef Dm
    dL_drot[4 * idx] = dq0; dL_drot[4 * idx + 1] = dq1; dL_drot[4 * idx + 2] = dq2; dL_drot[4 * idx + 3] = dq3;
  } else {
    dL_dscale[3 * idx] = 0.f; dL_dscale[3 * idx + 1] = 0.f; dL_dscale[3 * idx + 2] = 0.f;
    dL_drot[4 * idx] = 0.f; dL_drot[4 * idx + 1] = 0.f; dL_drot[4 * idx + 2] = 0.f; dL_drot[4 * idx + 3] = 0.f;
  }
}

template <bool STAGED, bool DEPTH = false>
__global__ __launch_bounds__(PRE_BLOCK) void k_gaussian_backward(
    const FrameParams fp, GeomState g, const int* __restrict__ radii, const float* __restrict__ means3D, const float* __restrict__ scales,
    const float* __restrict__ rotations, const float* __restrict__ shs, const float* __restrict__ cov3D_precomp,
    const float* __restrict__ V, const float* __restrict__ Pm, const float* __restrict__ campos,
    const int colors_are_precomp, float* dL_dmean2D, float* dL_dconic, float* dL_dopacity, float* dL_dcolor,
    float* __restrict__ dL_dmean3D,
    float* __restrict__ dL_dcov3D, float* __restrict__ dL_dsh, float* __restrict__ dL_dscale,
    float* __restrict__ dL_drot, const bool skip_recordless, float* dL_ddepths) {
  extern __shared__ float sh_rows[];
  __shared__ uint32_t s_rec[PRE_BLOCK];
  __shared__ uint32_t s_nrec;
  const int row0 = blockIdx.x * PRE_BLOCK, idx = row0 + threadIdx.x;
  const int C = fp.M * 3, nrows = min(PRE_BLOCK, fp.P - row0);
  if (STAGED) {
    if (threadIdx.x == 0) s_nrec = 0u;
    __syncthreads();
    if (idx < fp.P && radii[idx] > 0 && (g.touched[idx] != 0 || !skip_recordless)) s_rec[atomicAdd(&s_nrec, 1u)] = threadIdx.x;
    __syncthreads();
    listed_rows_to_lds(sh_rows, shs + (size_t)row0 * C, s_rec, (int)s_nrec, C);
    __syncthreads();
  }
  if (idx < fp.P)
    gaussian_backward_one<DEPTH>(idx, STAGED ? sh_rows + threadIdx.x * sh_row_stride(C) : nullptr, fp, g, radii, means3D,
                                 scales, rotations, shs, cov3D_precomp, V, Pm, campos, colors_are_precomp, dL_dmean2D,
                                 dL_dconic, dL_dopacity, dL_dcolor, dL_dmean3D, dL_dcov3D, dL_dsh, dL_dscale, dL_drot,
                                 dL_ddepths, skip_recordless);
  if (STAGED) {
    __syncthreads();
    lds_to_rows(dL_dsh + (size_t)row0 * C, sh_rows, nrows, C);
  }
}

__global__ __launch_bounds__(PRE_BLOCK) void k_mark_visible(int P, const float* __restrict__ means3D,
                                                            const float* __restrict__ V,
                                                            unsigned char* __restrict__ present) {
  const int idx = blockIdx.x * PRE_BLOCK + threadIdx.x;
  if (idx >= P) return;
  const float z = V[2] * means3D[3 * idx] + V[6] * means3D[3 * idx + 1] + V[10] * means3D[3 * idx + 2] + V[14];
  present[idx] = !(z <= 0.2f);
}

constexpr int POSE_ROWS = PRE_BLOCK;
constexpr int POSE_FINISH = 256;

__device__ __forceinline__ double wave_sum_f64(double v) {
#pragma unroll
  for (int o = 32; o > 0; o >>= 1) v += __shfl_xor(v, o, 64);
  return v;
}

__global__ __launch_bounds__(POSE_ROWS) void k_pose_partials(
    const FrameParams fp, const int* __restrict__ radii, const float* __restrict__ means3D,
    const float* __restrict__ scales, const float* __restrict__ rotations, const float* __restrict__ cov3D_precomp,
    const float* __restrict__ V, const float* __restrict__ Pm, const float* __restrict__ dL_dmean2D,
    const float* __restrict__ dL_dconic, const float* __restrict__ dL_ddepths, const float* __restrict__ dL_dmean3D,
    double* __restrict__ partials) {
  __shared__ double s_wave[POSE_ROWS / 64][6];
  const size_t idx = (size_t)blockIdx.x * POSE_ROWS + threadIdx.x;
  float term[6] = {0.f, 0.f, 0.f, 0.f, 0.f, 0.f};
  if (idx < (size_t)fp.P && radii[idx] > 0) {
    const float mx = means3D[3 * idx], my = means3D[3 * idx + 1], mz = means3D[3 * idx + 2];
    const float gmx = dL_dmean2D[3 * idx], gmy = dL_dmean2D[3 * idx + 1];
    const float gca = dL_dconic[4 * idx], gcb = dL_dconic[4 * idx + 1], gcc = dL_dconic[4 * idx + 3];
    const float gz = dL_ddepths ? dL_ddepths[idx] : 0.f;
    const float g0 = dL_dmean3D[3 * idx], g1 = dL_dmean3D[3 * idx + 1], g2 = dL_dmean3D[3 * idx + 2];
    float c6[6];
    if (cov3D_precomp) {
#pragma unroll
      for (int k = 0; k < 6; k++) c6[k] = cov3D_precomp[6 * idx + k];
    } else {
      const float4 q = reinterpret_cast<const float4*>(rotations)[idx];
      cov3d_from_scale_rot(fp.scale_modifier * scales[3 * idx], fp.scale_modifier * scales[3 * idx + 1],
                           fp.scale_modifier * scales[3 * idx + 2], q, c6);
    }
    float dcov[6];
    float gm0, gm1, gm2;
    geometric_backward(mx, my, mz, fp, c6, V, Pm, gmx, gmy, gca, gcb, gcc, nullptr, dcov, gm0, gm1, gm2);
    const float d0 = gm0 + V[2] * gz, d1 = gm1 + V[6] * gz, d2 = gm2 + V[10] * gz;
    term[0] = V[0] * g0 + V[4] * g1 + V[8] * g2;
    term[1] = V[1] * g0 + V[5] * g1 + V[9] * g2;
    term[2] = V[2] * g0 + V[6] * g1 + V[10] * g2;
    const float t0 = V[0] * mx + V[4] * my + V[8] * mz + V[12];
    const float t1 = V[1] * mx + V[5] * my + V[9] * mz + V[13];
    const float t2 = V[2] * mx + V[6] * my + V[10] * mz + V[14];
    const float r0 = V[0] * d0 + V[4] * d1 + V[8] * d2;
    const float r1 = V[1] * d0 + V[5] * d1 + V[9] * d2;
    const float r2 = V[2] * d0 + V[6] * d1 + V[10] * d2;
    const float Rm[3][3] = {{V[0], V[4], V[8]}, {V[1], V[5], V[9]}, {V[2], V[6], V[10]}};
    const float Sw[3][3] = {{c6[0], c6[1], c6[2]}, {c6[1], c6[3], c6[4]}, {c6[2], c6[4], c6[5]}};
    const float Gw[3][3] = {{dcov[0], 0.5f * dcov[1], 0.5f * dcov[2]},
                            {0.5f * dcov[1], dcov[3], 0.5f * dcov[4]},
                            {0.5f * dcov[2], 0.5f * dcov[4], dcov[5]}};
    float Sc[3][3], Gc[3][3];
#pragma unroll
    for (int i = 0; i < 3; i++) {
      float rs[3], rg[3];
#pragma unroll
      for (int k = 0; k < 3; k++) {
        rs[k] = Rm[i][0] * Sw[0][k] + Rm[i][1] * Sw[1][k] + Rm[i][2] * Sw[2][k];
        rg[k] = Rm[i][0] * Gw[0][k] + Rm[i][1] * Gw[1][k] + Rm[i][2] * Gw[2][k];
      }
#pragma unroll
      for (int j = 0; j < 3; j++) {
        Sc[i][j] = rs[0] * Rm[j][0] + rs[1] * Rm[j][1] + rs[2] * Rm[j][2];
        Gc[i][j] = rg[0] * Rm[j][0] + rg[1] * Rm[j][1] + rg[2] * Rm[j][2];
      }
    }
#define POSE_COMM(i, j) ((Gc[i][0] * Sc[0][j] + Gc[i][1] * Sc[1][j] + Gc[i][2] * Sc[2][j]) - \
                         (Sc[i][0] * Gc[0][j] + Sc[i][1] * Gc[1][j] + Sc[i][2] * Gc[2][j]))
    term[3] = (t1 * r2 - t2 * r1) + 2.f * POSE_COMM(2, 1);
    term[4] = (t2 * r0 - t0 * r2) + 2.f * POSE_COMM(0, 2);
    term[5] = (t0 * r1 - t1 * r0) + 2.f * POSE_COMM(1, 0);
// ... 99 lines not shown

hipError_t launch_compact_near(const FrameParams& fp, GeomState g, const uint32_t* top_hist, uint32_t near_budget,
                               uint32_t* keys_out, uint32_t* vals_out, uint32_t* n_out, uint32_t* ghist_near,
                               unsigned long long* publish, uint32_t ticket, hipStream_t s) {
  ProfScope ps(K_COMPACT_NEAR, s);
  hipLaunchKernelGGL(k_compact_near, dim3((fp.P + COMPACT_TILE - 1) / COMPACT_TILE), dim3(PRE_BLOCK), 0, s, fp.P, g.dkeysA,
                     top_hist, near_budget, keys_out, vals_out, n_out, ghist_near, g.dsort.scanC_status(),
                     g.dsort.tickets() + 6, publish, ticket);
  return hipGetLastError();
}

hipError_t launch_scan_offsets_far(const FrameParams& fp, GeomState g, Count capB, uint32_t slot_base, const uint32_t* sat,
                                   uint32_t* chunk_firstB, uint32_t* counts0, unsigned long long* publish,
                                   uint32_t ticket, hipStream_t s) {
  const size_t ncounts0 = (size_t)((capB.cap + TSORT_TILE - 1) / TSORT_TILE) * 256;
  ProfScope ps(K_SCAN_OFFSETS, s);
  hipLaunchKernelGGL(k_scan_offsets_far, dim3((fp.P + SCAN_TILE - 1) / SCAN_TILE), dim3(PRE_BLOCK), 0, s, fp, g, capB,
                     slot_base, sat, chunk_firstB, counts0, ncounts0, publish, ticket);
  return hipGetLastError();
}

hipError_t launch_emit(const FrameParams& fp, const uint4* sdesc, Count R, uint32_t* chunk_first, uint32_t* tkeys_out,
                       uint32_t* ivals_out, uint8_t* inst_flag, uint32_t* counts0, uint32_t digit_shift0,
                       uint32_t digit_mask0, bool key16, bool store_pairs, hipStream_t s) {
  if (R.cap <= 0) return hipSuccess;
  ProfScope ps(K_EMIT, s);
  const dim3 grid(chain_grid(R, EMIT_CHUNK));
  if (key16 && store_pairs)
    hipLaunchKernelGGL((k_emit<uint16_t, true>), grid, dim3(256), 0, s, fp, sdesc, R, chunk_first,
                       reinterpret_cast<uint16_t*>(tkeys_out), ivals_out, inst_flag, counts0, digit_shift0, digit_mask0);
  else if (key16)
    hipLaunchKernelGGL((k_emit<uint16_t, false>), grid, dim3(256), 0, s, fp, sdesc, R, chunk_first,
                       reinterpret_cast<uint16_t*>(tkeys_out), ivals_out, inst_flag, counts0, digit_shift0, digit_mask0);
  else
    hipLaunchKernelGGL((k_emit<uint32_t, true>), grid, dim3(256), 0, s, fp, sdesc, R, chunk_first, tkeys_out, ivals_out,
                       inst_flag, counts0, digit_shift0, digit_mask0);
  return hipGetLastError();
}

hipError_t launch_emit_scatter(const EmitFusion& ef, uint16_t* keys_out, uint32_t* vals_out, int shift0, int nbits0,
                               const uint32_t* counts, const uint32_t* chunk_base, const uint32_t* digit_total,
                               bool arank, hipStream_t s) {
  const dim3 grid(chain_grid(ef.R, TSORT_TILE));
  if (arank)
    hipLaunchKernelGGL(k_emit_scatter<true>, grid, dim3(256), 0, s, ef.fp, ef.sdesc, ef.R, ef.chunk_first, keys_out, vals_out,
                       shift0, nbits0, counts, chunk_base, digit_total);
  else
    hipLaunchKernelGGL(k_emit_scatter<false>, grid, dim3(256), 0, s, ef.fp, ef.sdesc, ef.R, ef.chunk_first, keys_out,
                       vals_out, shift0, nbits0, counts, chunk_base, digit_total);
  return hipGetLastError();
}

hipError_t launch_gather_records(const FrameParams& fp, GeomState g, BinningState b, float* dL_dmean2D,
                                 float* dL_dconic, float* dL_dopacity, float* dL_dcolor, float* dL_ddepths,
                                 bool split_frame, hipStream_t s) {
  const int nb = (fp.P + PRE_BLOCK - 1) / PRE_BLOCK;
  if (!split_frame) {
    ProfScope ps(K_COMPACT_TOUCHED, s);
    hipLaunchKernelGGL(k_compact_touched, dim3((nb + 15) / 16), dim3(PRE_BLOCK), 0, s, fp.P, g.touched, g.tlist,
                       g.total + 2);
  }
  {
    ProfScope ps(K_GATHER_RECORDS, s);
    const int want = (fp.P + PRE_BLOCK / 64 - 1) / (PRE_BLOCK / 64);
    const int grid = want < 4096 ? want : 4096;
    if (dL_ddepths)
      hipLaunchKernelGGL(k_gather_records<RecordSumsDepth>, dim3(grid), dim3(PRE_BLOCK), 0, s, g, b.grad_inst,
                         b.inst_flag, dL_dmean2D, dL_dconic, dL_dopacity, dL_dcolor, 0.5f * (float)fp.W,
                         0.5f * (float)fp.H, fp.P, split_frame, dL_ddepths);
    else
      hipLaunchKernelGGL(k_gather_records<>, dim3(grid), dim3(PRE_BLOCK), 0, s, g, b.grad_inst, b.inst_flag, dL_dmean2D,
                         dL_dconic, dL_dopacity, dL_dcolor, 0.5f * (float)fp.W, 0.5f * (float)fp.H, fp.P, split_frame,
                         nullptr);
  }
  return hipGetLastError();
}

hipError_t launch_gaussian_backward(const FrameParams& fp, GeomState g, BinningState b, const int* radii,
                                    const float* means3D, const float* scales, const float* rotations,
                                    const float* shs, const float* cov3D_precomp, const float* view, const float* proj,
                                    const float* campos, bool colors_precomp, float* dL_dmean2D, float* dL_dconic,
                                    float* dL_dopacity, float* dL_dcolor, float* dL_dmean3D, float* dL_dcov3D,
                                    float* dL_dsh, float* dL_dscale, float* dL_drot, float* dL_ddepths,
                                    hipStream_t s) {
  const int nb = (fp.P + PRE_BLOCK - 1) / PRE_BLOCK;
  ProfScope ps_k_gaussian_bwd(K_GAUSSIAN_BWD, s);
  const size_t stage = (shs && !colors_precomp) ? sh_stage_bytes(fp.M) : 0;
  const bool skip_recordless = !env().gbwd_all;
  if (dL_ddepths) {
    if (stage)
      hipLaunchKernelGGL((k_gaussian_backward<true, true>), dim3(nb), dim3(PRE_BLOCK), stage, s, fp, g, radii, means3D,
                         scales, rotations, shs, cov3D_precomp, view, proj, campos, 0, dL_dmean2D, dL_dconic, dL_dopacity,
                         dL_dcolor, dL_dmean3D, dL_dcov3D, dL_dsh, dL_dscale, dL_drot, skip_recordless, dL_ddepths);
    else
      hipLaunchKernelGGL((k_gaussian_backward<false, true>), dim3(nb), dim3(PRE_BLOCK), 0, s, fp, g, radii, means3D,
                         scales, rotations, shs, cov3D_precomp, view, proj, campos, colors_precomp ? 1 : 0, dL_dmean2D,
                         dL_dconic, dL_dopacity, dL_dcolor, dL_dmean3D, dL_dcov3D, dL_dsh, dL_dscale, dL_drot,
                         skip_recordless, dL_ddepths);
  } else if (stage)
    hipLaunchKernelGGL(k_gaussian_backward<true>, dim3(nb), dim3(PRE_BLOCK), stage, s, fp, g, radii,
                       means3D, scales, rotations, shs, cov3D_precomp, view, proj, campos, 0,
                       dL_dmean2D, dL_dconic, dL_dopacity, dL_dcolor, dL_dmean3D, dL_dcov3D, dL_dsh, dL_dscale, dL_drot,
                       skip_recordless, nullptr);
  else
    hipLaunchKernelGGL(k_gaussian_backward<false>, dim3(nb), dim3(PRE_BLOCK), 0, s, fp, g, radii,
                       means3D, scales, rotations, shs, cov3D_precomp, view, proj, campos, colors_precomp ? 1 : 0,
                       dL_dmean2D, dL_dconic, dL_dopacity, dL_dcolor, dL_dmean3D, dL_dcov3D, dL_dsh, dL_dscale, dL_drot,
                       skip_recordless, nullptr);
  return hipGetLastError();
}

hipError_t launch_mark_visible(int P, const float* means3D, const float* view, unsigned char* present,
                               hipStream_t s) {
  const int nb = (P + PRE_BLOCK - 1) / PRE_BLOCK;
  ProfScope ps_k_mark_visible(K_MARK_VISIBLE, s);
  hipLaunchKernelGGL(k_mark_visible, dim3(nb), dim3(PRE_BLOCK), 0, s, P, means3D, view, present);
  return hipGetLastError();
}

static inline size_t pose_partials(int P) { return ((size_t)P + POSE_ROWS - 1) / POSE_ROWS; }
size_t pose_workspace_bytes(int P) { return pose_partials(P) * 6 * sizeof(double) + 16; }

hipError_t launch_pose_gradient(const FrameParams& fp, const int* radii, const float* means3D, const float* scales,
                                const float* rotations, const float* cov3D_precomp, const float* view,
                                const float* proj, const float* dL_dmean2D, const float* dL_dconic,
                                const float* dL_ddepths, const float* dL_dmean3D, float* dL_dpose, char* workspace,
                                hipStream_t s) {
  double* partials = reinterpret_cast<double*>((reinterpret_cast<uintptr_t>(workspace) + 15u) & ~(uintptr_t)15u);
  const int nb = (int)pose_partials(fp.P);
  if (nb > 0) {
    ProfScope ps(K_POSE_PARTIALS, s);
    hipLaunchKernelGGL(k_pose_partials, dim3(nb), dim3(POSE_ROWS), 0, s, fp, radii, means3D, scales, rotations,
                       cov3D_precomp, view, proj, dL_dmean2D, dL_dconic, dL_ddepths, dL_dmean3D, partials);
    const hipError_t e = hipGetLastError();
    if (e != hipSuccess) return e;
  }
  ProfScope ps(K_POSE_FINISH, s);
  hipLaunchKernelGGL(k_pose_finish, dim3(1), dim3(POSE_FINISH), 0, s, nb, partials, dL_dpose);
  return hipGetLastError();
}

}
```

gs-livm_amd/csrc/render.hip:

```cpp
#include "gsr_internal.hpp"

namespace gsr {



template <int CTRL, int ROW_MASK, int BANK_MASK>
__device__ __forceinline__ float dpp_get(float v) {
  return __int_as_float(__builtin_amdgcn_update_dpp(0, __float_as_int(v), CTRL, ROW_MASK, BANK_MASK, false));
}

__device__ __forceinline__ float wave_sum_to_hi(float v) {
  v += __int_as_float(__builtin_amdgcn_update_dpp(__float_as_int(v), __float_as_int(v), 0xB1, 0xF, 0xF, true));
  v += __int_as_float(__builtin_amdgcn_update_dpp(__float_as_int(v), __float_as_int(v), 0x4E, 0xF, 0xF, true));
  v += __int_as_float(__builtin_amdgcn_update_dpp(__float_as_int(v), __float_as_int(v), 0x124, 0xF, 0xF, true));
  v += __int_as_float(__builtin_amdgcn_update_dpp(__float_as_int(v), __float_as_int(v), 0x128, 0xF, 0xF, true));
  v += dpp_get<0x142, 0xA, 0xF>(v);
  v += dpp_get<0x143, 0xC, 0xF>(v);
  return v;
}

__device__ __forceinline__ void swap_add32(float& a, float& b) {
  const auto r = __builtin_amdgcn_permlane32_swap(__float_as_uint(a), __float_as_uint(b), false, false);
  a = __uint_as_float(r[0]) + __uint_as_float(r[1]);
}
// ... 212 lines not shown
          "v_add_f32_e32 %[A], %[A], %[t0]\n\t"
          "v_mov_b32_e32 %[T], %[dx]\n\t"
          "v_mov_b32_e32 %[last], %[pos]\n\t"
          "s_mov_b64 exec, %[sv]"
          : [t0] "=&v"(t0), [t1] "=&v"(t1), [dx] "=&v"(dx), [dy] "=&v"(dy), [sv] "=&s"(sv), [done] "+s"(done_m),
            [C0] "+v"(C0), [C1] "+v"(C1), [C2] "+v"(C2), [Dp] "+v"(Dp), [A] "+v"(A), [T] "+v"(T), [last] "+v"(last)
          : [ax] "v"(ra.x), [ay] "v"(ra.y), [Aa] "v"(ra.z), [Bb] "v"(ra.w), [Cc] "v"(rb.x), [op] "v"(rb.y), [cr] "v"(rb.z),
            [cg] "v"(rb.w), [cb] "v"(rc.x), [dz] "v"(rc.y), [pos] "v"(rc.z), [pfx] "v"(pfx), [pfy] "v"(pfy)
          : "vcc", "scc");
    };
    if (nh) {
      if (lane == 0 && (nh & 1)) {
        sA[nh] = make_float4(0.f, 0.f, 0.f, 0.f);
        sB[nh] = make_float4(0.f, 0.f, 0.f, 0.f);
        sC[nh] = make_float4(0.f, 0.f, 0.f, 0.f);
      }
      const int nh2 = (nh + 1) & ~1;
      float4 a0 = sA[0], b0 = sB[0], c0 = sC[0];
      __builtin_amdgcn_s_waitcnt(0xC07F);
      for (int r = 0; r < nh2; r += 2) {
        const float4 a1 = sA[r + 1], b1 = sB[r + 1], c1 = sC[r + 1];
        visit(a0, b0, c0);
        __builtin_amdgcn_s_waitcnt(0xC07F);
        a0 = sA[r + 2]; b0 = sB[r + 2]; c0 = sC[r + 2];
        visit(a1, b1, c1);
        __builtin_amdgcn_s_waitcnt(0xC07F);
        if (done_m == ~0ull) {
          wave_done = true;
          break;
        }
      }
    }
  }

  done = ((done_m >> lane) & 1ull) != 0ull;
  const uint32_t wl = wave_max_u32(inside ? last : 0u);
  if (lane == 0) quad_last[quad] = wl;
  if (PHASE == 1) {
    const bool all_stopped = done_m == ~0ull;
    if (lane == 0) {
      quad_done[quad] = all_stopped ? 1 : 0;
      const uint32_t old = atomicAdd(&s_done, 1u | (all_stopped ? 0u : 0x100u));
      if ((old & 0xFFu) == (uint32_t)FW - 1u) {
        const uint32_t mine = (old >> 8) + (all_stopped ? 0u : 1u);
        const unsigned long long o = atomicAdd(done_word, (1ull << 40) | (unsigned long long)mine);
        if ((o >> 40) == (unsigned long long)gridDim.x - 1ull) {
          const uint32_t live = (uint32_t)((o & ((1ull << 40) - 1ull)) + mine);
          *live_quads_out = live;
          __hip_atomic_store(done_word, 0ull, __ATOMIC_RELAXED, __HIP_MEMORY_SCOPE_AGENT);
          if (publish)
            __hip_atomic_store(publish, ((unsigned long long)ticket << 32) | live, __ATOMIC_RELAXED,
                               __HIP_MEMORY_SCOPE_SYSTEM);
          if (aw.decide && live == 0u) {
            const uint32_t d = 2u * aw.seq;
            __hip_atomic_store(aw.gate_dev, d, __ATOMIC_RELAXED, __HIP_MEMORY_SCOPE_AGENT);
            __hip_atomic_store(aw.go, aw.seq, __ATOMIC_RELAXED, __HIP_MEMORY_SCOPE_SYSTEM);
            __hip_atomic_store(aw.decide, d, __ATOMIC_RELEASE, __HIP_MEMORY_SCOPE_SYSTEM);
          }
        }
      }
    }
    if (!all_stopped) {
      if (inside) {
        final_T[pid] = T;
        n_contrib[pid] = last | (done ? STOPPED_BIT : 0u);
        out_color[pid] = C0; out_color[N + pid] = C1; out_color[2 * N + pid] = C2;
        out_depth[pid] = Dp;
        out_acc[pid] = A;
      }
      return;
    }
  }
  if (inside) {
    final_T[pid] = T;
    n_contrib[pid] = last;
    out_color[pid] = C0 + T * bg[0];
    out_color[N + pid] = C1 + T * bg[1];
    out_color[2 * N + pid] = C2 + T * bg[2];
    out_depth[pid] = Dp;
    out_acc[pid] = A;
  }
}

template <int BCHUNK, bool DEPTH = false>
__global__ __launch_bounds__(256) void k_blend_backward(
    const FrameParams fp, const uint2* __restrict__ ranges, const uint32_t* __restrict__ quad_last_in,
    const uint32_t* __restrict__ point_list, const float4* __restrict__ splats, const uint2* __restrict__ slotinfo,
    const float* __restrict__ bg, const float* __restrict__ final_T, const uint32_t* __restrict__ n_contrib,
    const float* __restrict__ dL_dpix, const float* __restrict__ dL_dacc, float4* __restrict__ grad_inst,
    uint8_t* __restrict__ inst_flag, uint8_t* __restrict__ touched, const uint32_t* __restrict__ tile_order,
    const uint2* __restrict__ rangesB, const float* __restrict__ dL_ddepth) {
  constexpr int LW = BCHUNK / 64;
  constexpr int PF = DEPTH ? 16 : 12, RF = PF / 4;
  __shared__ float4 sE[BCHUNK][3];
  __shared__ uint32_t sSlot[BCHUNK], sId[BCHUNK];
  __shared__ uint64_t smask[4][LW];
  __shared__ __attribute__((aligned(16))) float sPart[4][BCHUNK][PF];
  const int tid = threadIdx.x, lane = tid & 63, w = tid >> 6;
  const int tile = tile_order ? (int)tile_order[blockIdx.x] : (int)blockIdx.x;
  const int tile_x = tile % fp.gx, tile_y = tile / fp.gx;
  const uint32_t ql0 = quad_last_in[4 * tile], ql1 = quad_last_in[4 * tile + 1], ql2 = quad_last_in[4 * tile + 2],
                 ql3 = quad_last_in[4 * tile + 3];
  const int n = (int)max(max(ql0, ql1), max(ql2, ql3));
  if (n == 0) return;
  const uint2 rng = ranges[tile];
  const uint32_t rbase = rng.x, rbaseB = rangesB[tile].x;
  const int lenA = (int)(rng.y - rng.x);
  const int px = tile_x * TILE + (w & 1) * 8 + (lane & 7);
  const int py = tile_y * TILE + (w >> 1) * 8 + (lane >> 3);
  const bool inside = px < fp.W && py < fp.H;
  const float pfx = (float)px, pfy = (float)py;
  const float tx0 = (float)(tile_x * TILE), ty0 = (float)(tile_y * TILE);
  const size_t pid = (size_t)fp.W * py + px, N = (size_t)fp.W * fp.H;

  const float T_final = inside ? final_T[pid] : 0.0f;
  const int lastc = inside ? (int)n_contrib[pid] : 0;
  const float dp0 = inside ? dL_dpix[pid] : 0.f, dp1 = inside ? dL_dpix[N + pid] : 0.f,
              dp2 = inside ? dL_dpix[2 * N + pid] : 0.f;
  const float dacc = inside ? dL_dacc[pid] : 0.f;
  float ddep = 0.f;
  if constexpr (DEPTH) ddep = inside ? dL_ddepth[pid] : 0.f;
  float T = T_final;
  float S = bg[0] * dp0 + bg[1] * dp1 + bg[2] * dp2;

  float* const my_part = &sPart[w][0][0] + RF * (lane >> 4);
  for (int base = 0; base < n; base += BCHUNK) {
    const int k = base + tid;
    const bool stager = tid < BCHUNK;
    uint32_t hits = 0;
    if (stager && k < n) {
      const int pos = n - 1 - k;
      const uint32_t id = pos < lenA ? point_list[rbase + pos] : point_list[rbaseB + (uint32_t)(pos - lenA)];
      const float4 a = splats[(size_t)id * SPLAT_F4 + 0];
      const float4 b = splats[(size_t)id * SPLAT_F4 + 1];
      const float4 c = splats[(size_t)id * SPLAT_F4 + 2];
      const uint2 si = slotinfo[id];
      const int x0 = (int)(si.y & 1023u), y0 = (int)((si.y >> 10) & 1023u), rw = (int)(si.y >> 20);
      constexpr float L2E = 1.4426950408889634f;
      sE[tid][0] = make_float4(a.x, a.y, a.z * (-0.5f * L2E), a.w * (-L2E));
      sE[tid][1] = make_float4(b.x * (-0.5f * L2E), b.y, b.z, b.w);
      if constexpr (DEPTH) sE[tid][2] = make_float4(c.x, c.y, a.w, b.x);
      else sE[tid][2] = make_float4(c.x, a.z, a.w, b.x);
      sId[tid] = id;
      sSlot[tid] = si.x + (uint32_t)((tile_y - y0) * rw + (tile_x - x0));
      hits = quad_hits(a.x, a.y, c.z, c.w, tx0, ty0);
      if (hits && c.z < 1.0e6f) {
        const float tau = footprint_tau(b.y);
#pragma unroll
        for (int q = 0; q < 4; q++)
          if (((hits >> q) & 1u) &&
              !ellipse_reaches_quad(a.x, a.y, a.z, a.w, b.x, tau, tx0 + (float)((q & 1) * 8), ty0 + (float)((q >> 1) * 8)))
            hits &= ~(1u << q);
      }
      hits &= (pos < (int)ql0 ? 1u : 0u) | (pos < (int)ql1 ? 2u : 0u) | (pos < (int)ql2 ? 4u : 0u) |
              (pos < (int)ql3 ? 8u : 0u);
    }
    if (w < LW) {
#pragma unroll
      for (int q = 0; q < 4; q++) {
        const uint64_t m = __ballot((hits >> q) & 1u);
        if (lane == 0) smask[q][w] = m;
      }
    }
    __syncthreads();
    for (int lw = 0; lw < LW; lw++) {
      uint64_t m = uniform_u64(smask[w][lw]);
      while (m) {
        const int bpos = __builtin_ctzll(m);
        m &= m - 1;
        const int jj = lw * 64 + bpos;
        const int pos = n - 1 - (base + jj);
        const float4 a = sE[jj][0];
        const float4 b = sE[jj][1];
        const float blue = sE[jj][2].x;
        float dacc_z = dacc;
        if constexpr (DEPTH) dacc_z = __builtin_fmaf(sE[jj][2].y, ddep, dacc);
        const float dx = a.x - pfx, dy = a.y - pfy;
        const float power = splat_power(a.z, a.w, b.x, dx, dy);
        const float Graw = __builtin_amdgcn_exp2f(power);
        const float araw = fminf(0.99f, b.y * Graw);
        const bool ok = (pos < lastc) && !(power > 0.0f) && !(araw < 1.0f / 255.0f);
        const float alpha = ok ? araw : 0.0f;
        const float oma = 1.0f - alpha;
        const float rom = __builtin_amdgcn_rcpf(oma);
        const float Tn = T * rom;
        const float Draw = __builtin_fmaf(b.z, dp0, __builtin_fmaf(b.w, dp1, __builtin_fmaf(blue, dp2, dacc_z))) - S;
        const float D = ok ? Draw : 0.0f;
        if (__ballot(ok) != 0ull) {
          const float G = ok ? Graw : 0.0f;
          const float dch = alpha * Tn;
          const float dL_dalpha = Tn * D;
          const float dLG = G * dL_dalpha;
          const float sx = dLG * dx, sy = dLG * dy;
          const float g0 = dch * dp0, g1 = dch * dp1, g2 = dch * dp2;
          const float g3 = sx, g4 = sy;
          const float g5 = sx * dx, g6 = sx * dy, g7 = sy * dy;
          float g8 = dLG;
          float w0, w1;
          wave_sum8(g0, g1, g2, g3, g4, g5, g6, g7, w0, w1);
          g8 = row_allsum(g8);
          asm volatile("" : "+v"(w0), "+v"(w1), "+v"(g8));
          float g9 = 0.f;
          if constexpr (DEPTH) g9 = row_allsum(dch * ddep);
          if ((lane & 15) == 0) {
            float* const dst = my_part + (uint32_t)PF * (uint32_t)jj;
            dst[0] = w0; dst[1] = w1; dst[2] = g8;
            if constexpr (DEPTH) dst[3] = g9;
          }
        } else if ((lane & 15) == 0) {
          float* const dst = my_part + (uint32_t)PF * (uint32_t)jj;
          dst[0] = 0.f; dst[1] = 0.f; dst[2] = 0.f;
          if constexpr (DEPTH) dst[3] = 0.f;
        }
        T = Tn;
        S = __builtin_fmaf(alpha, D, S);
      }
    }
    __syncthreads();
    if (stager && k < n) {
      const int lw = tid >> 6;
      float s[9] = {0, 0, 0, 0, 0, 0, 0, 0, 0};
      float s9 = 0.f;
      bool any = false;
#pragma unroll
      for (int q = 0; q < 4; q++) {
        if ((smask[q][lw] >> (tid & 63)) & 1ull) {
          any = true;
#pragma unroll
          for (int r = 0; r < 4; r++) {
            s[2 * r] += sPart[q][tid][RF * r];
            s[2 * r + 1] += sPart[q][tid][RF * r + 1];
          }
          s[8] += (sPart[q][tid][2] + sPart[q][tid][RF + 2]) + (sPart[q][tid][2 * RF + 2] + sPart[q][tid][3 * RF + 2]);
          if constexpr (DEPTH)
            s9 += (sPart[q][tid][3] + sPart[q][tid][RF + 3]) + (sPart[q][tid][2 * RF + 3] + sPart[q][tid][3 * RF + 3]);
        }
      }
      if (any) {
        const size_t slot = sSlot[tid];
        grad_inst[slot * GRAD_F4 + 0] = make_float4(s[0], s[1], s[2], s[3]);
        grad_inst[slot * GRAD_F4 + 1] = make_float4(s[4], s[5], s[6], s[7]);
        grad_inst[slot * GRAD_F4 + 2] = make_float4(s[8], 0.f, DEPTH ? s9 : 0.f, 0.f);
        inst_flag[slot] = 1;
        touched[sId[tid]] = 1;
      }
    }
    __syncthreads();
  }
}

__global__ __launch_bounds__(1024) void k_tile_order(const uint32_t* __restrict__ quad_last, const int T,
                                                     uint32_t* __restrict__ order) {
  __shared__ uint32_t bins[1024];
  __shared__ uint32_t wtot[16];
  const int tid = threadIdx.x, lane = tid & 63, w = tid >> 6;
  bins[tid] = 0u;
  __syncthreads();
  auto walk = [&](int t) {
    const uint4 q = *reinterpret_cast<const uint4*>(quad_last + 4 * (size_t)t);
    const uint32_t m = max(max(q.x, q.y), max(q.z, q.w));
    return m < 1023u ? m : 1023u;
  };
  uint32_t wk[8];
#pragma unroll
  for (int k = 0; k < 8; k++) wk[k] = tid + 1024 * k < T ? walk(tid + 1024 * k) : 0u;
#pragma unroll
  for (int k = 0; k < 8; k++)
    if (tid + 1024 * k < T) atomicAdd(&bins[wk[k]], 1u);
  for (int t = tid + 8192; t < T; t += 1024) atomicAdd(&bins[walk(t)], 1u);
  __syncthreads();
  const uint32_t v = bins[1023 - tid];
  uint32_t inc = v;
#pragma unroll
  for (int o = 1; o < 64; o <<= 1) {
    const uint32_t u = __shfl_up(inc, o, 64);
    if (lane >= o) inc += u;
  }
  if (lane == 63) wtot[w] = inc;
  __syncthreads();
  uint32_t base = inc - v;
  for (int k = 0; k < w; k++) base += wtot[k];
  bins[1023 - tid] = base;
  __syncthreads();
#pragma unroll
  for (int k = 0; k < 8; k++)
    if (tid + 1024 * k < T) order[atomicAdd(&bins[wk[k]], 1u)] = (uint32_t)(tid + 1024 * k);
  for (int t = tid + 8192; t < T; t += 1024) order[atomicAdd(&bins[walk(t)], 1u)] = (uint32_t)t;
}

template <int TW, bool DEPTH = false>
__global__ __launch_bounds__(64 * TW, 1) void k_blend_backward_tile(
    const FrameParams fp, const uint2* __restrict__ ranges, const uint32_t* __restrict__ quad_last_in,
    const uint32_t* __restrict__ point_list, const float4* __restrict__ splats, const uint2* __restrict__ slotinfo,
    const float* __restrict__ bg, const float* __restrict__ final_T, const uint32_t* __restrict__ n_contrib,
    const float* __restrict__ dL_dpix, const float* __restrict__ dL_dacc, float* __restrict__ grad_inst,
    uint8_t* __restrict__ inst_flag, uint8_t* __restrict__ touched, const uint32_t* __restrict__ tile_order,
    const uint2* __restrict__ rangesB, const float* __restrict__ dL_ddepth) {
  __shared__ float4 sE[TW][64][3];
  __shared__ uint32_t sSlot[TW][64], sId[TW][64];
  const int lane = threadIdx.x & 63, wq = __builtin_amdgcn_readfirstlane(threadIdx.x >> 6);
  if (blockIdx.x * TW + wq >= fp.gx * fp.gy) return;
  const int tile = __builtin_amdgcn_readfirstlane(tile_order ? (int)tile_order[blockIdx.x * TW + wq]
                                                             : (int)(blockIdx.x * TW + wq));
  const uint32_t ql0 = quad_last_in[4 * tile], ql1 = quad_last_in[4 * tile + 1], ql2 = quad_last_in[4 * tile + 2],
                 ql3 = quad_last_in[4 * tile + 3];
  const int n = __builtin_amdgcn_readfirstlane((int)max(max(ql0, ql1), max(ql2, ql3)));
  if (n == 0) return;
  const int tile_x = tile % fp.gx, tile_y = tile / fp.gx;
  const uint2 rng = ranges[tile];
  const uint32_t rbase = rng.x, rbaseB = rangesB[tile].x;
  const int lenA = (int)(rng.y - rng.x);
  const int px = tile_x * TILE + (lane & 15);
  const float pfx = (float)px;
  const float tx0 = (float)(tile_x * TILE), ty0 = (float)(tile_y * TILE);
  const size_t N = (size_t)fp.W * fp.H;
  const float bg0 = bg[0], bg1 = bg[1], bg2 = bg[2];

  float pfy[4], T[4], S[4], dp0[4], dp1[4], dp2[4], dacc[4];
  float ddep[4] = {0.f, 0.f, 0.f, 0.f};
  int lastc[4];
#pragma unroll
  for (int k = 0; k < 4; k++) {
    const int py = tile_y * TILE + 4 * k + (lane >> 4);
    const bool inside = px < fp.W && py < fp.H;
    const size_t pid = (size_t)fp.W * py + px;
    pfy[k] = (float)py;
    T[k] = inside ? final_T[pid] : 0.0f;
    lastc[k] = inside ? (int)n_contrib[pid] : 0;
    dp0[k] = inside ? dL_dpix[pid] : 0.f;
    dp1[k] = inside ? dL_dpix[N + pid] : 0.f;
    dp2[k] = inside ? dL_dpix[2 * N + pid] : 0.f;
    dacc[k] = inside ? dL_dacc[pid] : 0.f;
    if constexpr (DEPTH) ddep[k] = inside ? dL_ddepth[pid] : 0.f;
    S[k] = bg0 * dp0[k] + bg1 * dp1[k] + bg2 * dp2[k];
  }

  float4 a = make_float4(0, 0, 0, 0), b = a, c = a;
  uint32_t eid = 0, eslot = 0;
  bool hit = false;
  auto gather = [&](const int k) {
    hit = false;
    if (k < n) {
      const int pos = n - 1 - k;
      const uint32_t id = pos < lenA ? point_list[rbase + (uint32_t)pos] : point_list[rbaseB + (uint32_t)(pos - lenA)];
      a = splats[(size_t)id * SPLAT_F4 + 0];
      b = splats[(size_t)id * SPLAT_F4 + 1];
      c = splats[(size_t)id * SPLAT_F4 + 2];
      const uint2 si = slotinfo[id];
      const int x0 = (int)(si.y & 1023u), y0 = (int)((si.y >> 10) & 1023u), rw = (int)(si.y >> 20);
      eid = id;
      eslot = si.x + (uint32_t)((tile_y - y0) * rw + (tile_x - x0));
      hit = (a.x + c.z >= tx0) && (a.x - c.z <= tx0 + 15.0f) && (a.y + c.w >= ty0) && (a.y - c.w <= ty0 + 15.0f);
      if (hit && c.z < 1.0e6f)
        hit = ellipse_reaches_quad<15>(a.x, a.y, a.z, a.w, b.x, footprint_tau(b.y), tx0, ty0);
    }
  };
  gather(lane);
  float* const rec_lane = grad_inst + 2 * (lane >> 4);
  for (int base = 0; base < n; base += 64) {
    constexpr float L2E = 1.4426950408889634f;
    sE[wq][lane][0] = make_float4(a.x, a.y, a.z * (-0.5f * L2E), a.w * (-L2E));
    sE[wq][lane][1] = make_float4(b.x * (-0.5f * L2E), b.y, b.z, b.w);
    sE[wq][lane][2] = make_float4(c.x, DEPTH ? c.y : 0.f, 0.f, 0.f);
    sSlot[wq][lane] = eslot;
    sId[wq][lane] = eid;
    uint64_t m = __ballot(hit);
    gather(base + 64 + lane);
    while (m) {
      const int jj = __builtin_ctzll(m);
      m &= m - 1;
      const int pos = n - 1 - (base + jj);
      const float4 ea = sE[wq][jj][0];
      const float4 eb = sE[wq][jj][1];
      const float blue = sE[wq][jj][2].x;
      float ez = 0.f;
      if constexpr (DEPTH) ez = sE[wq][jj][2].y;
      const float dx = ea.x - pfx;
      const float dx2 = dx * dx;
      const float Adx2 = ea.z * dx2;
      float c0 = 0.f, c1 = 0.f, c2 = 0.f, sG = 0.f, sGy = 0.f, sGyy = 0.f;
      float sZ = 0.f;
      uint64_t anym = 0ull;
#pragma unroll
      for (int k = 0; k < 4; k++) {
        const float dy = ea.y - pfy[k];
        const float power = splat_power_shared(Adx2, ea.w, eb.x, dx, dy);
        const float Graw = __builtin_amdgcn_exp2f(power);
        const float araw = fminf(0.99f, eb.y * Graw);
        const bool ok = (pos < lastc[k]) && !(power > 0.0f) && !(araw < 1.0f / 255.0f);
        anym |= __builtin_amdgcn_ballot_w64(pos < lastc[k]) & __builtin_amdgcn_ballot_w64(!(power > 0.0f)) &
                __builtin_amdgcn_ballot_w64(!(araw < 1.0f / 255.0f));
        if (ok) {
          const float rom = __builtin_amdgcn_rcpf(1.0f - araw);
          const float Tn = T[k] * rom;
          float dacc_z = dacc[k];
          if constexpr (DEPTH) dacc_z = __builtin_fmaf(ez, ddep[k], dacc[k]);
          const float D =
              __builtin_fmaf(eb.z, dp0[k], __builtin_fmaf(eb.w, dp1[k], __builtin_fmaf(blue, dp2[k], dacc_z))) - S[k];
          const float dch = araw * Tn;
          const float dL_dalpha = Tn * D;
          const float dLG = Graw * dL_dalpha;
          const float sy = dLG * dy;
          c0 = __builtin_fmaf(dch, dp0[k], c0);
          c1 = __builtin_fmaf(dch, dp1[k], c1);
          c2 = __builtin_fmaf(dch, dp2[k], c2);
          if constexpr (DEPTH) sZ = __builtin_fmaf(dch, ddep[k], sZ);
          sG += dLG;
          sGy += sy;
          sGyy = __builtin_fmaf(sy, dy, sGyy);
          T[k] = Tn;
          S[k] = __builtin_fmaf(araw, D, S[k]);
        }
      }
      if (anym != 0ull) {
        float v0 = c0, v1 = c1, v2 = c2, v3 = dx * sG, v4 = sGy, v5 = dx2 * sG, v6 = dx * sGy, v7 = sGyy, g8 = sG;
        swap_add32(v0, v4);
        swap_add32(v1, v5);
        swap_add32(v2, v6);
        swap_add32(v3, v7);
        swap_add16(v0, v2);
        swap_add16(v1, v3);
        row_allsum3(v0, v1, g8);
        asm volatile("" : "+v"(v0), "+v"(v1), "+v"(g8));
        if constexpr (DEPTH) {
          float g9 = row_allsum(sZ);
          swap_add16(g8, g9);
        }
        const size_t slot = sSlot[wq][jj];
        if ((lane & 15) == 0) {
          *reinterpret_cast<float2*>(rec_lane + slot * (GRAD_F4 * 4)) = make_float2(v0, v1);
          if constexpr (DEPTH) grad_inst[slot * (GRAD_F4 * 4) + 8 + (lane >> 5) + 2 * ((lane >> 4) & 1)] = g8;
          else grad_inst[slot * (GRAD_F4 * 4) + 8 + (lane >> 4)] = g8;
        }
        if (lane == 63) {
          inst_flag[slot] = 1;
          touched[sId[wq][jj]] = 1;
        }
      }
    }
  }
}

template <bool IN_LDS>
__global__ __launch_bounds__(1024) void k_live_sat(const uint8_t* __restrict__ quad_done, const int gx, const int gy,
                                                   uint32_t* __restrict__ sat, uint32_t* __restrict__ total_live,
                                                   const Count gate) {
  extern __shared__ uint32_t s_sat[];
  if (gate.closed()) return;
  uint32_t* const S = IN_LDS ? s_sat : sat;
  const int sw = gx + 1, tid = threadIdx.x, lane = tid & 63, w = tid >> 6;
  if (IN_LDS) {
    for (int i = tid; i < sw * (gy + 1); i += 1024) {
      const int y = i / sw - 1, x = i % sw - 1;
      uint32_t live = 0;
      if (x >= 0 && y >= 0) {
        const uchar4 q = *reinterpret_cast<const uchar4*>(quad_done + 4 * ((size_t)y * gx + x));
        live = (q.x & q.y & q.z & q.w) ? 0u : 1u;
      }
      S[i] = live;
    }
    __syncthreads();
    for (int y = w; y < gy; y += 16) {
      uint32_t carry = 0;
      for (int x0 = 0; x0 < gx; x0 += 64) {
        const int x = x0 + lane;
        uint32_t v = x < gx ? S[(y + 1) * sw + x + 1] : 0u;
#pragma unroll
        for (int o = 1; o < 64; o <<= 1) {
          const uint32_t u = __shfl_up(v, o, 64);
          if (lane >= o) v += u;
        }
        if (x < gx) S[(y + 1) * sw + x + 1] = carry + v;
        carry += __shfl(v, 63, 64);
      }
    }
    __syncthreads();
  } else {
    for (int i = tid; i < sw; i += 1024) S[i] = 0u;
    for (int y = tid; y < gy; y += 1024) {
      uint32_t run = 0;
      S[(y + 1) * sw] = 0u;
      for (int x = 0; x < gx; x++) {
        const uchar4 q = *reinterpret_cast<const uchar4*>(quad_done + 4 * ((size_t)y * gx + x));
        run += (q.x & q.y & q.z & q.w) ? 0u : 1u;
        S[(y + 1) * sw + x + 1] = run;
      }
    }
    __syncthreads();
  }
  for (int x = tid; x < gx; x += 1024) {
    uint32_t run = 0;
    for (int y = 0; y < gy; y++) {
      run += S[(y + 1) * sw + x + 1];
      S[(y + 1) * sw + x + 1] = run;
    }
  }
  __syncthreads();
  if (IN_LDS)
    for (int i = tid; i < sw * (gy + 1); i += 1024) sat[i] = S[i];
  if (tid == 0) *total_live = S[gy * sw + gx];
}

__global__ void k_decide_far(const uint32_t* __restrict__ live_quads, const AsyncWords aw) {
  if (threadIdx.x != 0 || *live_quads == 0u) return;
  const uint32_t d = 2u * aw.seq + 1u;
  __hip_atomic_store(aw.gate_dev, d, __ATOMIC_RELAXED, __HIP_MEMORY_SCOPE_AGENT);
  __hip_atomic_store(aw.decide, d, __ATOMIC_RELEASE, __HIP_MEMORY_SCOPE_SYSTEM);
}
hipError_t launch_decide_far(const uint32_t* live_quads, AsyncWords aw, hipStream_t s) {
  hipLaunchKernelGGL(k_decide_far, dim3(1), dim3(64), 0, s, live_quads, aw);
  return hipGetLastError();
}

__global__ void k_release_go(const Count gate, uint32_t* __restrict__ go, const uint32_t seq) {
  if (threadIdx.x == 0 && !gate.closed()) __hip_atomic_store(go, seq, __ATOMIC_RELAXED, __HIP_MEMORY_SCOPE_SYSTEM);
}
hipError_t launch_release_go(Count gate, uint32_t* go, uint32_t seq, hipStream_t s) {
  hipLaunchKernelGGL(k_release_go, dim3(1), dim3(64), 0, s, gate, go, seq);
  return hipGetLastError();
}

hipError_t launch_live_sat(const FrameParams& fp, ImageState im, uint32_t* total_live, Count gate, hipStream_t s) {
  ProfScope ps(K_LIVE_SAT, s);
  const size_t bytes = (size_t)(fp.gx + 1) * (fp.gy + 1) * sizeof(uint32_t);
  if (bytes <= 150 * 1024) {
    static const hipError_t attr = hipFuncSetAttribute(reinterpret_cast<const void*>(&k_live_sat<true>),
                                                       hipFuncAttributeMaxDynamicSharedMemorySize, 150 * 1024);
    if (attr != hipSuccess) return attr;
    hipLaunchKernelGGL(k_live_sat<true>, dim3(1), dim3(1024), bytes, s, im.quad_done, fp.gx, fp.gy, im.live_sat,
                       total_live, gate);
  } else {
    hipLaunchKernelGGL(k_live_sat<false>, dim3(1), dim3(1024), 0, s, im.quad_done, fp.gx, fp.gy, im.live_sat, total_live,
                       gate);
  }
  return hipGetLastError();
}

hipError_t launch_blend_forward(const FrameParams& fp, GeomState g, BinningState b, ImageState im, const float* bg,
                                float* out_color, float* out_depth, float* out_acc, int phase,
                                unsigned long long* done_word, unsigned long long* publish, uint32_t ticket,
                                AsyncWords aw, Count gate, hipStream_t s) {
  ProfScope ps_k_blend_fwd(K_BLEND_FWD, s);
  const int quads = fp.gx * fp.gy * 4;
#define GSR_LAUNCH_FWD(PH)                                                                                            \
  hipLaunchKernelGGL((k_blend_forward<4, PH>), dim3((quads + 3) / 4), dim3(256), 0, s, fp, im.ranges, im.rangesB,      \
                     b.point_list, g.splats, bg, im.final_T, im.n_contrib, im.quad_last, im.quad_done, out_color,      \
                     out_depth, out_acc, done_word, publish, ticket, g.total + 13, aw, gate)
  if (phase == 1) GSR_LAUNCH_FWD(1);
  else if (phase == 2) GSR_LAUNCH_FWD(2);
  else GSR_LAUNCH_FWD(0);
#undef GSR_LAUNCH_FWD
  return hipGetLastError();
}

hipError_t launch_tile_order(const FrameParams& fp, ImageState im, hipStream_t s) {
  if (env().bwd_image_order) return hipSuccess;
  ProfScope ps(K_TILE_ORDER, s);
  hipLaunchKernelGGL(k_tile_order, dim3(1), dim3(1024), 0, s, im.quad_last, fp.gx * fp.gy, im.tile_order);
  return hipGetLastError();
}

hipError_t launch_blend_backward(const FrameParams& fp, GeomState g, BinningState b, ImageState im, const float* bg,
                                 const float* dL_dpix, const float* dL_dacc, const float* dL_ddepth, bool have_tile_order,
                                 hipStream_t s) {
  if (!have_tile_order) {
    const hipError_t e = launch_tile_order(fp, im, s);
    if (e != hipSuccess) return e;
  }
  ProfScope ps_k_blend_bwd(K_BLEND_BWD, s);
  const int tiles = fp.gx * fp.gy;
  const bool per_quad = env().blend_backward_quads || (!env().blend_backward_tiles && tiles < 3072);
  const uint32_t* order = env().bwd_image_order ? nullptr : im.tile_order;
  constexpr int TW = 4;
  if (dL_ddepth) {
    if (per_quad)
      hipLaunchKernelGGL((k_blend_backward<128, true>), dim3(tiles), dim3(256), 0, s, fp, im.ranges, im.quad_last,
                         b.point_list, g.splats, g.slotinfo, bg, im.final_T, im.n_contrib, dL_dpix, dL_dacc, b.grad_inst,
                         b.inst_flag, g.touched, order, im.rangesB, dL_ddepth);
    else
      hipLaunchKernelGGL((k_blend_backward_tile<TW, true>), dim3((tiles + TW - 1) / TW), dim3(64 * TW), 0, s, fp,
                         im.ranges, im.quad_last, b.point_list, g.splats, g.slotinfo, bg, im.final_T, im.n_contrib, dL_dpix,
                         dL_dacc, reinterpret_cast<float*>(b.grad_inst), b.inst_flag, g.touched, order, im.rangesB,
                         dL_ddepth);
  } else if (per_quad) {
    hipLaunchKernelGGL(k_blend_backward<128>, dim3(tiles), dim3(256), 0, s, fp, im.ranges, im.quad_last, b.point_list,
                       g.splats, g.slotinfo, bg, im.final_T, im.n_contrib, dL_dpix, dL_dacc, b.grad_inst, b.inst_flag,
                       g.touched, order, im.rangesB, nullptr);
  } else {
    hipLaunchKernelGGL(k_blend_backward_tile<TW>, dim3((tiles + TW - 1) / TW), dim3(64 * TW), 0, s, fp, im.ranges,
                       im.quad_last, b.point_list, g.splats, g.slotinfo, bg, im.final_T, im.n_contrib, dL_dpix, dL_dacc,
                       reinterpret_cast<float*>(b.grad_inst), b.inst_flag, g.touched, order, im.rangesB, nullptr);
  }
  return hipGetLastError();
}

}
```

include/gsraster.h:

```cpp
#ifndef GSRASTER_H_INCLUDED
#define GSRASTER_H_INCLUDED

#include <stddef.h>
#include <stdint.h>

#ifdef __cplusplus
extern "C" {
#endif

#define GSR_ABI_VERSION 2

typedef enum gsr_status {
  GSR_OK = 0,
  GSR_ERR_INVALID_ARGUMENT = -1,
  GSR_ERR_ALLOC = -2,
  GSR_ERR_HIP = -3,
  GSR_ERR_UNSUPPORTED = -4
} gsr_status;

typedef char* (*gsr_alloc_fn)(void* ctx, size_t bytes);


int gsr_forward(gsr_alloc_fn geometry_alloc, void* geometry_ctx, gsr_alloc_fn binning_alloc, void* binning_ctx,
                gsr_alloc_fn image_alloc, void* image_ctx, int P, int D, int M, const float* background, int width,
                int height, const float* means3D, const float* shs, const float* colors_precomp,
                const float* opacities, const float* scales, float scale_modifier, const float* rotations,
                const float* cov3D_precomp, const float* viewmatrix, const float* projmatrix, const float* cam_pos,
                float tan_fovx, float tan_fovy, int prefiltered, float* out_color, float* out_depth, float* out_acc,
                int* radii, int debug, void* stream);

int gsr_last_num_rendered(void);
long long gsr_set_binning_capacity_hint(long long capacity);
unsigned long long gsr_speculative_forwards(void);
unsigned long long gsr_speculation_overflows(void);
unsigned long long gsr_emit_guard_trips(void);

int gsr_set_near_far(int on);
int gsr_set_near_far_thread(int mode);
int gsr_near_far(void);
int gsr_last_near_far(unsigned* near_instances, unsigned* far_instances);
void gsr_set_near_far_hints(long long near_entries_per_tile, long long far_capacity);
unsigned long long gsr_near_far_forwards(void);
int gsr_set_far_speculation(int mode);
int gsr_last_far_skipped(void);
unsigned long long gsr_far_skips(void);
unsigned long long gsr_far_skip_misses(void);
unsigned long long gsr_async_far_frames(void);
int gsr_async_outcomes_pending(void);
unsigned long long gsr_async_outcomes_lost(void);
unsigned long long gsr_frame_note_misses(void);
unsigned gsr_near_budget_scale(void);
unsigned gsr_near_budget_feedback(unsigned unfinished_quads, unsigned near_instances, unsigned far_instances);
int gsr_near_far_pause(int frames);

int gsr_backward(int P, int D, int M, int R, const float* background, int width, int height, const float* means3D,
                 const float* shs, const float* colors_precomp, const float* scales, float scale_modifier,
                 const float* rotations, const float* cov3D_precomp, const float* viewmatrix,
                 const float* projmatrix, const float* campos, float tan_fovx, float tan_fovy, const int* radii,
                 char* geom_buffer, char* binning_buffer, char* image_buffer, const float* dL_dpix,
                 const float* dL_dacc, float* dL_dmean2D, float* dL_dconic, float* dL_dopacity, float* dL_dcolor,
                 float* dL_dmean3D, float* dL_dcov3D, float* dL_dsh, float* dL_dscale, float* dL_drot, int debug,
                 void* stream);

int gsr_backward_depth(int P, int D, int M, int R, const float* background, int width, int height,
                       const float* means3D, const float* shs, const float* colors_precomp, const float* scales,
                       float scale_modifier, const float* rotations, const float* cov3D_precomp,
                       const float* viewmatrix, const float* projmatrix, const float* campos, float tan_fovx,
                       float tan_fovy, const int* radii, char* geom_buffer, char* binning_buffer, char* image_buffer,
                       const float* dL_dpix, const float* dL_dacc, const float* dL_ddepth, float* dL_dmean2D,
                       float* dL_dconic, float* dL_dopacity, float* dL_dcolor, float* dL_dmean3D, float* dL_dcov3D,
                       float* dL_dsh, float* dL_dscale, float* dL_drot, float* dL_ddepths, int debug, void* stream);

size_t gsr_pose_gradient_workspace(int P);
int gsr_pose_gradient(int P, int width, int height, const float* means3D, const float* scales, float scale_modifier,
                      const float* rotations, const float* cov3D_precomp, const float* viewmatrix,
                      const float* projmatrix, float tan_fovx, float tan_fovy, const int* radii,
                      const float* dL_dmean2D, const float* dL_dconic, const float* dL_ddepths ,
                      const float* dL_dmean3D, float* dL_dpose , char* workspace, size_t workspace_bytes,
                      void* stream);

int gsr_mark_visible(int P, const float* means3D, const float* viewmatrix, const float* projmatrix,
                     unsigned char* present, void* stream);

size_t gsr_geometry_bytes(int P);
size_t gsr_image_bytes(int width, int height);
size_t gsr_binning_bytes(int R);

typedef struct gsr_geometry_view {
  const float* depths;
  const int32_t* radii;
  const float* splats;
  const float* cov3D;
  const uint32_t* tiles_touched;
  const uint32_t* point_offsets;
  const uint8_t* clamped;
  const uint32_t* depth_order;
  const uint32_t* num_rendered;
  const uint32_t* gpack;
} gsr_geometry_view;
typedef struct gsr_binning_view {
  const uint32_t* point_list;
} gsr_binning_view;
typedef struct gsr_image_view {
  const uint32_t* ranges;
  const float* final_T;
  const uint32_t* n_contrib;
  const uint32_t* quad_last;
  const uint32_t* ranges_far;
} gsr_image_view;
int gsr_geometry_view_of(char* geom_buffer, int P, gsr_geometry_view* out);
int gsr_binning_view_of(char* binning_buffer, int R, gsr_binning_view* out);
int gsr_image_view_of(char* image_buffer, int width, int height, gsr_image_view* out);

int gsr_set_reference_rects(int on);
int gsr_set_reference_rects_thread(int mode);
int gsr_reference_rects(void);

uint32_t gsr_higher_msb(uint32_t n);

int gsr_activate(int P, int M, const float* scaling_raw, const float* rotation_raw, const float* opacity_raw,
                 const float* features_dc, const float* features_rest, float* scales, float* rotations,
                 float* opacities, float* shs, void* stream);
int gsr_activate_backward(int P, int M, const float* rotation_raw, const float* scales, const float* opacities,
                          const float* dL_dscales, const float* dL_drotations, const float* dL_dopacities,
                          const float* dL_dshs, float* dL_dscaling_raw, float* dL_drotation_raw,
                          float* dL_dopacity_raw, float* dL_dfeatures_dc, float* dL_dfeatures_rest, void* stream);
int gsr_model_step(int P, int M, float* const* params6, float* const* exp_avg6, float* const* exp_avg_sq6,
                   const float* dL_dxyz, const float* dL_dscales, const float* dL_drotations, const float* dL_dopacities,
                   const float* dL_dshs, float* scales_out, float* rotations_out, float* opacities_out, float* shs_out,
                   const float* lr6, double beta1, double beta2, double eps, int step, void* stream);
int gsr_adam_step(int n_tensors, float* const* params, float* const* grads, float* const* exp_avg,
                  float* const* exp_avg_sq, const size_t* numel, const float* lr, double beta1, double beta2, double eps,
                  int step, int zero_grads, void* stream);
// ... 105 lines not shown
```

Measured before the change: 1174 Mpixels/s.

## Zero untouched gradient rows inside blend-backward waves instead of gaussian-backward

Moves the zeroing of per-Gaussian gradient buffers into the blend-backward kernel, where each wave clears a slice of the buffers once it finishes (or exits early) its tile work. The gaussian-backward kernel then skips rows for untouched Gaussians and writes SH gradients only for listed rows. The aim is to overlap the bulk zero-fill with the compute-heavy blend pass and to drop per-thread scalar stores for the many invisible Gaussians. The cost is extra store traffic appended to blend-backward waves and more complex correctness conditions. The path is enabled by default unless GSR_BWD_FILL is zero.

```diff
diff --git a/gs-livm_amd/__init__.py b/gs-livm_amd/__init__.py
--- a/gs-livm_amd/__init__.py
+++ b/gs-livm_amd/__init__.py
@@ -1,6 +1,6 @@
 from . import multiview, synthetic
 from ._capi import (GsrError, LIB_PATH, NumRendered, emit_guard_trips, last_num_rendered, lib, mailbox_slow_path_last, mark_visible,
-                    set_binning_capacity_hint, speculation_stats, set_near_far, set_near_far_thread, set_reference_rects_thread, async_outcomes_pending, set_near_far_hints, last_near_far, set_far_speculation, last_far_skipped, profile_enable, profile_read,
+                    set_binning_capacity_hint, speculation_stats, set_near_far, set_near_far_thread, set_reference_rects_thread, async_outcomes_pending, set_near_far_hints, last_near_far, set_far_speculation, last_far_skipped, profile_enable, profile_read, set_backward_fill, backward_fills,
                     pose_gradient, rasterize_backward, rasterize_forward, reference_rects, set_reference_rects, state_views)
 from .loss import (DeltaDepthLoss, ExposureLoss, LidarDepthLoss, PhotometricLoss, SimilarityLoss, delta_depth_loss, delta_pose,
                    apply_exposure, exposure_photometric_loss, identity_exposure, lidar_depth_image, lidar_depth_loss,
@@ -32,4 +32,4 @@
 
 
 __all__ = ["KeyframeVisibility", "visibility_pack", "covisibility", "observation_count", "visibility_remap", "iou", "overlap_coefficient", "ExposureLoss", "exposure_photometric_loss", "apply_exposure", "identity_exposure", "LidarDepthLoss", "lidar_depth_image", "lidar_depth_loss", "raster_K", "world_to_camera", "prune_rows", "image_metrics", "psnr", "to_u8", "side_by_side", "depth_to_u8", "evaluate_keyframes", "DeltaDepthLoss", "delta_depth_loss", "delta_pose", "SimilarityLoss", "similarity_loss", "VoxelIndex", "PhotometricLoss", "photometric_loss", "reference_window_1d", "FusedActivations", "FusedAdam", "GaussianParameters", "GrowableAdam", "GrowableGaussians", "ply", "GaussianRasterizationSettings", "GaussianRasterizer", "rasterize_gaussians", "Camera", "render", "render_full", "se3_exp", "pose_gradient", "get_projection_matrix", "rasterize_forward",
-           "rasterize_backward", "mark_visible", "state_views", "set_reference_rects", "reference_rects", "last_num_rendered", "set_binning_capacity_hint", "speculation_stats", "emit_guard_trips", "mailbox_slow_path_last", "set_near_far", "set_near_far_thread", "set_reference_rects_thread", "async_outcomes_pending", "set_near_far_hints", "last_near_far", "set_far_speculation", "last_far_skipped", "NumRendered", "lib", "torch_ops", "synthetic", "multiview", "GsrError", "LIB_PATH"]
+           "rasterize_backward", "mark_visible", "state_views", "set_reference_rects", "reference_rects", "last_num_rendered", "set_binning_capacity_hint", "speculation_stats", "emit_guard_trips", "mailbox_slow_path_last", "set_near_far", "set_near_far_thread", "set_reference_rects_thread", "async_outcomes_pending", "set_near_far_hints", "last_near_far", "set_far_speculation", "last_far_skipped", "set_backward_fill", "backward_fills", "NumRendered", "lib", "torch_ops", "synthetic", "multiview", "GsrError", "LIB_PATH"]
diff --git a/gs-livm_amd/_capi.py b/gs-livm_amd/_capi.py
--- a/gs-livm_amd/_capi.py
+++ b/gs-livm_amd/_capi.py
@@ -63,7 +63,8 @@
            "gsr_lidar_depth_loss_workspace", "gsr_density_accumulate", "gsr_densify_workspace", "gsr_densify_mark",
            "gsr_densify_apply", "gsr_pose_gradient", "gsr_pose_gradient_workspace", "gsr_exposure_loss",
            "gsr_exposure_loss_workspace", "gsr_apply_exposure", "gsr_visibility_words", "gsr_visibility_pack",
-           "gsr_covisibility", "gsr_observation_count", "gsr_visibility_remap")
+           "gsr_covisibility", "gsr_observation_count", "gsr_visibility_remap", "gsr_set_backward_fill",
+           "gsr_backward_fills")
 
 
 def lib():
@@ -147,6 +148,10 @@
         getattr(L, n).argtypes = [ci]
     L.gsr_async_outcomes_pending.restype = ci
     L.gsr_async_outcomes_pending.argtypes = []
+    L.gsr_set_backward_fill.restype = ci
+    L.gsr_set_backward_fill.argtypes = [ci]
+    L.gsr_backward_fills.restype = C.c_ulonglong
+    L.gsr_backward_fills.argtypes = []
     L.gsr_mailbox_slow_path_last.restype = ci
     L.gsr_mailbox_slow_path_last.argtypes = [C.POINTER(MailboxEvent)]
     L.gsr_mailbox_slow_path_hits.restype = C.c_ulonglong
@@ -431,6 +436,14 @@
     return split, int(a.value), int(b.value)
 
 
+def set_backward_fill(on):
+    return bool(lib().gsr_set_backward_fill(int(bool(on))))
+
+
+def backward_fills():
+    return int(lib().gsr_backward_fills())
+
+
 def set_reference_rects(on):
     return bool(lib().gsr_set_reference_rects(int(bool(on))))
 
diff --git a/gs-livm_amd/csrc/api.hip b/gs-livm_amd/csrc/api.hip
--- a/gs-livm_amd/csrc/api.hip
+++ b/gs-livm_amd/csrc/api.hip
@@ -63,6 +63,7 @@
     x.blend_backward_tiles = set(getenv("GSR_BLEND_BACKWARD_TILES"));
     x.bwd_image_order = set(getenv("GSR_BWD_IMAGE_ORDER"));
     x.gbwd_all = set(getenv("GSR_GBWD_ALL"));
+    x.bwd_fill = not_zero(getenv("GSR_BWD_FILL"));
     x.host_trace = set(getenv("GSR_HOST_TRACE"));
     return x;
   }();
@@ -1187,6 +1188,14 @@
 
 unsigned long long gsr_mailbox_slow_path_hits(void) { return g_mailbox_slow_hits.load(); }
 
+static std::atomic<int>& backward_fill_flag() {
+  static std::atomic<int> f{env().bwd_fill ? 1 : 0};
+  return f;
+}
+static std::atomic<unsigned long long> g_backward_fills{0};
+int gsr_set_backward_fill(int on) { return backward_fill_flag().exchange(on != 0 ? 1 : 0); }
+unsigned long long gsr_backward_fills(void) { return g_backward_fills.load(); }
+
 static int backward_impl(bool with_depth, int P, int D, int M, int R, const float* background, int width, int height,
                          const float* means3D, const float* shs, const float* colors_precomp, const float* scales,
                          float scale_modifier, const float* rotations, const float* cov3D_precomp,
@@ -1222,9 +1231,36 @@
   ImageState im = ImageState::carve(image_buffer, width, height);
   if (!radii) radii = g.radii;
 
+  GradFill fill;
+  if (R > 0 && !env().gbwd_all && backward_fill_flag().load(std::memory_order_relaxed) != 0) {
+    const size_t n = (size_t)P;
+    fill.add(dL_dmean2D, 3 * n);
+    fill.add(dL_dconic, 4 * n);
+    fill.add(dL_dopacity, n);
+    fill.add(dL_dcolor, 3 * n);
+    fill.add(dL_dmean3D, 3 * n);
+    fill.add(dL_dcov3D, 6 * n);
+    fill.add(dL_dsh, 3 * n * (size_t)M);
+    fill.add(dL_dscale, 3 * n);
+    fill.add(dL_drot, 4 * n);
+    if (with_depth) fill.add(dL_ddepths, n);
+    bool ok = true;
+    for (int i = 0; i < fill.n; i++) ok = ok && !misaligned16(fill.p[i]);
+    fill.waves = blend_backward_waves(fp);
+    const unsigned long long groups = fill.end[fill.n - 1];
+    const unsigned long long per_wave = (groups + fill.waves - 1) / fill.waves;
+    if (ok && per_wave * 16ull <= 64ull * 1024ull) {
+      fill.per_wave = (uint32_t)per_wave;
+      ++g_backward_fills;
+    } else {
+      fill.n = 0;
+    }
+  }
+  const bool rows_prefilled = fill.n != 0;
+
   if (R > 0) {
     const unsigned notes = frame_notes(image_buffer);
-    STAGE(launch_blend_backward(fp, g, b, im, background, dL_dpix, dL_dacc, dL_ddepth, (notes & NOTE_ORDER) != 0u,
+    STAGE(launch_blend_backward(fp, g, b, im, background, dL_dpix, dL_dacc, dL_ddepth, (notes & NOTE_ORDER) != 0u, fill,
                                 stream));
     STAGE(launch_gather_records(fp, g, b, dL_dmean2D, dL_dconic, dL_dopacity, dL_dcolor, dL_ddepths,
                                 (notes & NOTE_SPLIT) != 0u, stream));
@@ -1232,7 +1268,7 @@
   STAGE(launch_gaussian_backward(fp, g, b, radii, means3D, scales, rotations, colors_precomp ? nullptr : shs,
                                  cov3D_precomp, viewmatrix, projmatrix, campos, colors_precomp != nullptr, dL_dmean2D,
                                  dL_dconic, dL_dopacity, dL_dcolor, dL_dmean3D, dL_dcov3D, dL_dsh, dL_dscale, dL_drot,
-                                 dL_ddepths, stream));
+                                 dL_ddepths, rows_prefilled, stream));
   return GSR_OK;
 }
 
diff --git a/gs-livm_amd/csrc/gsr_internal.hpp b/gs-livm_amd/csrc/gsr_internal.hpp
--- a/gs-livm_amd/csrc/gsr_internal.hpp
+++ b/gs-livm_amd/csrc/gsr_internal.hpp
@@ -244,6 +244,7 @@
   bool blend_backward_tiles;
   bool bwd_image_order;
   bool gbwd_all;
+  bool bwd_fill;
   bool host_trace;
 };
 const Env& env();
@@ -314,16 +315,32 @@
 hipError_t launch_release_go(Count gate, uint32_t* go, uint32_t seq, hipStream_t s);
 hipError_t launch_decide_far(const uint32_t* live_quads, AsyncWords aw, hipStream_t s);
 hipError_t launch_tile_order(const FrameParams& fp, ImageState im, hipStream_t s);
+struct GradFill {
+  static constexpr int MAXA = 10;
+  float* p[MAXA];
+  unsigned long long end[MAXA];
+  uint32_t tail[MAXA];
+  int n = 0;
+  uint32_t waves = 0, per_wave = 0;
+  void add(float* q, size_t numel) {
+    if (!q || numel == 0) return;
+    p[n] = q;
+    end[n] = (n ? end[n - 1] : 0ull) + numel / 4;
+    tail[n] = (uint32_t)(numel & 3);
+    n++;
+  }
+};
+uint32_t blend_backward_waves(const FrameParams& fp);
 hipError_t launch_blend_backward(const FrameParams& fp, GeomState g, BinningState b, ImageState im, const float* bg,
                                  const float* dL_dpix, const float* dL_dacc, const float* dL_ddepth, bool have_tile_order,
-                                 hipStream_t s);
+                                 const GradFill& fill, hipStream_t s);
 hipError_t launch_gaussian_backward(const FrameParams& fp, GeomState g, BinningState b, const int* radii,
                                     const float* means3D, const float* scales, const float* rotations,
                                     const float* shs, const float* cov3D_precomp, const float* view, const float* proj,
                                     const float* campos, bool colors_precomp, float* dL_dmean2D, float* dL_dconic,
                                     float* dL_dopacity, float* dL_dcolor, float* dL_dmean3D, float* dL_dcov3D,
                                     float* dL_dsh, float* dL_dscale, float* dL_drot, float* dL_ddepths,
-                                    hipStream_t s);
+                                    bool rows_prefilled, hipStream_t s);
 hipError_t launch_mark_visible(int P, const float* means3D, const float* view, unsigned char* present, hipStream_t s);
 size_t pose_workspace_bytes(int P);
 hipError_t launch_pose_gradient(const FrameParams& fp, const int* radii, const float* means3D, const float* scales,
diff --git a/gs-livm_amd/csrc/preprocess.hip b/gs-livm_amd/csrc/preprocess.hip
--- a/gs-livm_amd/csrc/preprocess.hip
+++ b/gs-livm_amd/csrc/preprocess.hip
@@ -159,6 +159,24 @@
     for (int k = threadIdx.x; k < nlist * C; k += PRE_BLOCK) {
       const int r = (int)list[k / C], c = k % C;
       lds[r * S + c] = src[(size_t)r * C + c];
+    }
+  }
+}
+
+__device__ __forceinline__ void lds_to_listed_rows(float* __restrict__ dst, const float* lds, const uint32_t* list,
+                                                   const int nlist, const int C) {
+  const int S = sh_row_stride(C);
+  if ((C & 3) == 0 && (reinterpret_cast<uintptr_t>(dst) & 15u) == 0) {
+    const int C4 = C >> 2;
+    for (int k = threadIdx.x; k < nlist * C4; k += PRE_BLOCK) {
+      const int r = (int)list[k / C4], c4 = k % C4;
+      const float* d = lds + r * S + 4 * c4;
+      reinterpret_cast<float4*>(dst + (size_t)r * C)[c4] = make_float4(d[0], d[1], d[2], d[3]);
+    }
+  } else {
+    for (int k = threadIdx.x; k < nlist * C; k += PRE_BLOCK) {
+      const int r = (int)list[k / C], c = k % C;
+      dst[(size_t)r * C + c] = lds[r * S + c];
     }
   }
 }
@@ -1363,7 +1381,7 @@
     const int colors_are_precomp, float* dL_dmean2D, float* dL_dconic, float* dL_dopacity, float* dL_dcolor,
     float* __restrict__ dL_dmean3D,
     float* __restrict__ dL_dcov3D, float* __restrict__ dL_dsh, float* __restrict__ dL_dscale,
-    float* __restrict__ dL_drot, float* dL_ddepths, const bool skip_recordless) {
+    float* __restrict__ dL_drot, float* dL_ddepths, const bool skip_recordless, const bool rows_prefilled) {
   const int rad_in = radii[idx];
   const uint8_t touched_in = g.touched[idx];
   const bool vis = rad_in > 0;
@@ -1374,6 +1392,7 @@
   if (was_touched) g.touched[idx] = 0;
   const bool rec = vis && was_touched;
   if (!rec && (skip_recordless || !vis)) {
+    if (rows_prefilled && !was_touched) return;
     dL_dmean2D[3 * idx] = 0.f; dL_dmean2D[3 * idx + 1] = 0.f; dL_dmean2D[3 * idx + 2] = 0.f;
     dL_dconic[4 * idx] = 0.f; dL_dconic[4 * idx + 1] = 0.f; dL_dconic[4 * idx + 2] = 0.f; dL_dconic[4 * idx + 3] = 0.f;
     dL_dopacity[idx] = 0.f;
@@ -1552,7 +1571,7 @@
     const int colors_are_precomp, float* dL_dmean2D, float* dL_dconic, float* dL_dopacity, float* dL_dcolor,
     float* __restrict__ dL_dmean3D,
     float* __restrict__ dL_dcov3D, float* __restrict__ dL_dsh, float* __restrict__ dL_dscale,
-    float* __restrict__ dL_drot, const bool skip_recordless, float* dL_ddepths) {
+    float* __restrict__ dL_drot, const bool skip_recordless, float* dL_ddepths, const bool rows_prefilled) {
   extern __shared__ float sh_rows[];
   __shared__ uint32_t s_rec[PRE_BLOCK];
   __shared__ uint32_t s_nrec;
@@ -1561,7 +1580,8 @@
   if (STAGED) {
     if (threadIdx.x == 0) s_nrec = 0u;
     __syncthreads();
-    if (idx < fp.P && radii[idx] > 0 && (g.touched[idx] != 0 || !skip_recordless)) s_rec[atomicAdd(&s_nrec, 1u)] = threadIdx.x;
+    if (idx < fp.P && (rows_prefilled ? g.touched[idx] != 0 : radii[idx] > 0 && (g.touched[idx] != 0 || !skip_recordless)))
+      s_rec[atomicAdd(&s_nrec, 1u)] = threadIdx.x;
     __syncthreads();
     listed_rows_to_lds(sh_rows, shs + (size_t)row0 * C, s_rec, (int)s_nrec, C);
     __syncthreads();
@@ -1570,10 +1590,11 @@
     gaussian_backward_one<DEPTH>(idx, STAGED ? sh_rows + threadIdx.x * sh_row_stride(C) : nullptr, fp, g, radii, means3D,
                                  scales, rotations, shs, cov3D_precomp, V, Pm, campos, colors_are_precomp, dL_dmean2D,
                                  dL_dconic, dL_dopacity, dL_dcolor, dL_dmean3D, dL_dcov3D, dL_dsh, dL_dscale, dL_drot,
-                                 dL_ddepths, skip_recordless);
+                                 dL_ddepths, skip_recordless, rows_prefilled);
   if (STAGED) {
     __syncthreads();
-    lds_to_rows(dL_dsh + (size_t)row0 * C, sh_rows, nrows, C);
+    if (rows_prefilled) lds_to_listed_rows(dL_dsh + (size_t)row0 * C, sh_rows, s_rec, (int)s_nrec, C);
+    else lds_to_rows(dL_dsh + (size_t)row0 * C, sh_rows, nrows, C);
   }
 }
 
@@ -1839,7 +1860,7 @@
                                     const float* campos, bool colors_precomp, float* dL_dmean2D, float* dL_dconic,
                                     float* dL_dopacity, float* dL_dcolor, float* dL_dmean3D, float* dL_dcov3D,
                                     float* dL_dsh, float* dL_dscale, float* dL_drot, float* dL_ddepths,
-                                    hipStream_t s) {
+                                    bool rows_prefilled, hipStream_t s) {
   const int nb = (fp.P + PRE_BLOCK - 1) / PRE_BLOCK;
   ProfScope ps_k_gaussian_bwd(K_GAUSSIAN_BWD, s);
   const size_t stage = (shs && !colors_precomp) ? sh_stage_bytes(fp.M) : 0;
@@ -1848,22 +1869,22 @@
     if (stage)
       hipLaunchKernelGGL((k_gaussian_backward<true, true>), dim3(nb), dim3(PRE_BLOCK), stage, s, fp, g, radii, means3D,
                          scales, rotations, shs, cov3D_precomp, view, proj, campos, 0, dL_dmean2D, dL_dconic, dL_dopacity,
-                         dL_dcolor, dL_dmean3D, dL_dcov3D, dL_dsh, dL_dscale, dL_drot, skip_recordless, dL_ddepths);
+                         dL_dcolor, dL_dmean3D, dL_dcov3D, dL_dsh, dL_dscale, dL_drot, skip_recordless, dL_ddepths, rows_prefilled);
     else
       hipLaunchKernelGGL((k_gaussian_backward<false, true>), dim3(nb), dim3(PRE_BLOCK), 0, s, fp, g, radii, means3D,
                          scales, rotations, shs, cov3D_precomp, view, proj, campos, colors_precomp ? 1 : 0, dL_dmean2D,
                          dL_dconic, dL_dopacity, dL_dcolor, dL_dmean3D, dL_dcov3D, dL_dsh, dL_dscale, dL_drot,
-                         skip_recordless, dL_ddepths);
+                         skip_recordless, dL_ddepths, rows_prefilled);
   } else if (stage)
     hipLaunchKernelGGL(k_gaussian_backward<true>, dim3(nb), dim3(PRE_BLOCK), stage, s, fp, g, radii,
                        means3D, scales, rotations, shs, cov3D_precomp, view, proj, campos, 0,
                        dL_dmean2D, dL_dconic, dL_dopacity, dL_dcolor, dL_dmean3D, dL_dcov3D, dL_dsh, dL_dscale, dL_drot,
-                       skip_recordless, nullptr);
+                       skip_recordless, nullptr, rows_prefilled);
   else
     hipLaunchKernelGGL(k_gaussian_backward<false>, dim3(nb), dim3(PRE_BLOCK), 0, s, fp, g, radii,
                        means3D, scales, rotations, shs, cov3D_precomp, view, proj, campos, colors_precomp ? 1 : 0,
                        dL_dmean2D, dL_dconic, dL_dopacity, dL_dcolor, dL_dmean3D, dL_dcov3D, dL_dsh, dL_dscale, dL_drot,
-                       skip_recordless, nullptr);
+                       skip_recordless, nullptr, rows_prefilled);
   return hipGetLastError();
 }
 
diff --git a/gs-livm_amd/csrc/render.hip b/gs-livm_amd/csrc/render.hip
--- a/gs-livm_amd/csrc/render.hip
+++ b/gs-livm_amd/csrc/render.hip
@@ -318,6 +318,24 @@
   }
 }
 
+__device__ __forceinline__ void zero_fill_slice(const GradFill& f, const uint32_t wave, const int lane) {
+  const unsigned long long lo = (unsigned long long)wave * f.per_wave, hi = lo + f.per_wave;
+  const bool last_wave = wave == f.waves - 1u;
+  unsigned long long first = 0ull;
+#pragma unroll 1
+  for (int i = 0; i < f.n; i++) {
+    const unsigned long long end = f.end[i];
+    const unsigned long long a = lo > first ? lo : first, b = hi < end ? hi : end;
+    if (a < b) {
+      float4* dst = reinterpret_cast<float4*>(f.p[i]) + (a - first);
+      const uint32_t cnt = (uint32_t)(b - a);
+      for (uint32_t j = (uint32_t)lane; j < cnt; j += 64u) dst[j] = make_float4(0.f, 0.f, 0.f, 0.f);
+    }
+    if (last_wave && (uint32_t)lane < f.tail[i]) f.p[i][4ull * (end - first) + (uint32_t)lane] = 0.f;
+    first = end;
+  }
+}
+
 template <int BCHUNK, bool DEPTH = false>
 __global__ __launch_bounds__(256) void k_blend_backward(
     const FrameParams fp, const uint2* __restrict__ ranges, const uint32_t* __restrict__ quad_last_in,
@@ -325,7 +343,7 @@
     const float* __restrict__ bg, const float* __restrict__ final_T, const uint32_t* __restrict__ n_contrib,
     const float* __restrict__ dL_dpix, const float* __restrict__ dL_dacc, float4* __restrict__ grad_inst,
     uint8_t* __restrict__ inst_flag, uint8_t* __restrict__ touched, const uint32_t* __restrict__ tile_order,
-    const uint2* __restrict__ rangesB, const float* __restrict__ dL_ddepth) {
+    const uint2* __restrict__ rangesB, const float* __restrict__ dL_ddepth, const GradFill fill) {
   constexpr int LW = BCHUNK / 64;
   constexpr int PF = DEPTH ? 16 : 12, RF = PF / 4;
   __shared__ float4 sE[BCHUNK][3];
@@ -338,7 +356,11 @@
   const uint32_t ql0 = quad_last_in[4 * tile], ql1 = quad_last_in[4 * tile + 1], ql2 = quad_last_in[4 * tile + 2],
                  ql3 = quad_last_in[4 * tile + 3];
   const int n = (int)max(max(ql0, ql1), max(ql2, ql3));
-  if (n == 0) return;
+  const uint32_t fill_wave = blockIdx.x * 4u + (uint32_t)__builtin_amdgcn_readfirstlane(w);
+  if (n == 0) {
+    zero_fill_slice(fill, fill_wave, lane);
+    return;
+  }
   const uint2 rng = ranges[tile];
   const uint32_t rbase = rng.x, rbaseB = rangesB[tile].x;
   const int lenA = (int)(rng.y - rng.x);
@@ -483,6 +505,7 @@
     }
     __syncthreads();
   }
+  zero_fill_slice(fill, fill_wave, lane);
 }
 
 __global__ __launch_bounds__(1024) void k_tile_order(const uint32_t* __restrict__ quad_last, const int T,
@@ -531,17 +554,23 @@
     const float* __restrict__ bg, const float* __restrict__ final_T, const uint32_t* __restrict__ n_contrib,
     const float* __restrict__ dL_dpix, const float* __restrict__ dL_dacc, float* __restrict__ grad_inst,
     uint8_t* __restrict__ inst_flag, uint8_t* __restrict__ touched, const uint32_t* __restrict__ tile_order,
-    const uint2* __restrict__ rangesB, const float* __restrict__ dL_ddepth) {
+    const uint2* __restrict__ rangesB, const float* __restrict__ dL_ddepth, const GradFill fill) {
   __shared__ float4 sE[TW][64][3];
   __shared__ uint32_t sSlot[TW][64], sId[TW][64];
   const int lane = threadIdx.x & 63, wq = __builtin_amdgcn_readfirstlane(threadIdx.x >> 6);
-  if (blockIdx.x * TW + wq >= fp.gx * fp.gy) return;
+  if (blockIdx.x * TW + wq >= fp.gx * fp.gy) {
+    zero_fill_slice(fill, blockIdx.x * TW + wq, lane);
+    return;
+  }
   const int tile = __builtin_amdgcn_readfirstlane(tile_order ? (int)tile_order[blockIdx.x * TW + wq]
                                                              : (int)(blockIdx.x * TW + wq));
   const uint32_t ql0 = quad_last_in[4 * tile], ql1 = quad_last_in[4 * tile + 1], ql2 = quad_last_in[4 * tile + 2],
                  ql3 = quad_last_in[4 * tile + 3];
   const int n = __builtin_amdgcn_readfirstlane((int)max(max(ql0, ql1), max(ql2, ql3)));
-  if (n == 0) return;
+  if (n == 0) {
+    zero_fill_slice(fill, blockIdx.x * TW + wq, lane);
+    return;
+  }
   const int tile_x = tile % fp.gx, tile_y = tile / fp.gx;
   const uint2 rng = ranges[tile];
   const uint32_t rbase = rng.x, rbaseB = rangesB[tile].x;
@@ -675,6 +704,7 @@
       }
     }
   }
+  zero_fill_slice(fill, blockIdx.x * TW + wq, lane);
 }
 
 template <bool IN_LDS>
@@ -796,36 +826,45 @@
   return hipGetLastError();
 }
 
+constexpr int BWD_TW = 4;
+static bool blend_backward_per_quad(const FrameParams& fp) {
+  return env().blend_backward_quads || (!env().blend_backward_tiles && fp.gx * fp.gy < 3072);
+}
+uint32_t blend_backward_waves(const FrameParams& fp) {
+  const int tiles = fp.gx * fp.gy;
+  return blend_backward_per_quad(fp) ? 4u * (uint32_t)tiles : (uint32_t)((tiles + BWD_TW - 1) / BWD_TW * BWD_TW);
+}
+
 hipError_t launch_blend_backward(const FrameParams& fp, GeomState g, BinningState b, ImageState im, const float* bg,
                                  const float* dL_dpix, const float* dL_dacc, const float* dL_ddepth, bool have_tile_order,
-                                 hipStream_t s) {
+                                 const GradFill& fill, hipStream_t s) {
   if (!have_tile_order) {
     const hipError_t e = launch_tile_order(fp, im, s);
     if (e != hipSuccess) return e;
   }
   ProfScope ps_k_blend_bwd(K_BLEND_BWD, s);
   const int tiles = fp.gx * fp.gy;
-  const bool per_quad = env().blend_backward_quads || (!env().blend_backward_tiles && tiles < 3072);
+  const bool per_quad = blend_backward_per_quad(fp);
   const uint32_t* order = env().bwd_image_order ? nullptr : im.tile_order;
-  constexpr int TW = 4;
+  constexpr int TW = BWD_TW;
   if (dL_ddepth) {
     if (per_quad)
       hipLaunchKernelGGL((k_blend_backward<128, true>), dim3(tiles), dim3(256), 0, s, fp, im.ranges, im.quad_last,
                          b.point_list, g.splats, g.slotinfo, bg, im.final_T, im.n_contrib, dL_dpix, dL_dacc, b.grad_inst,
-                         b.inst_flag, g.touched, order, im.rangesB, dL_ddepth);
+                         b.inst_flag, g.touched, order, im.rangesB, dL_ddepth, fill);
     else
       hipLaunchKernelGGL((k_blend_backward_tile<TW, true>), dim3((tiles + TW - 1) / TW), dim3(64 * TW), 0, s, fp,
                          im.ranges, im.quad_last, b.point_list, g.splats, g.slotinfo, bg, im.final_T, im.n_contrib, dL_dpix,
                          dL_dacc, reinterpret_cast<float*>(b.grad_inst), b.inst_flag, g.touched, order, im.rangesB,
-                         dL_ddepth);
+                         dL_ddepth, fill);
   } else if (per_quad) {
     hipLaunchKernelGGL(k_blend_backward<128>, dim3(tiles), dim3(256), 0, s, fp, im.ranges, im.quad_last, b.point_list,
                        g.splats, g.slotinfo, bg, im.final_T, im.n_contrib, dL_dpix, dL_dacc, b.grad_inst, b.inst_flag,
-                       g.touched, order, im.rangesB, nullptr);
+                       g.touched, order, im.rangesB, nullptr, fill);
   } else {
     hipLaunchKernelGGL(k_blend_backward_tile<TW>, dim3((tiles + TW - 1) / TW), dim3(64 * TW), 0, s, fp, im.ranges,
                        im.quad_last, b.point_list, g.splats, g.slotinfo, bg, im.final_T, im.n_contrib, dL_dpix, dL_dacc,
-                       reinterpret_cast<float*>(b.grad_inst), b.inst_flag, g.touched, order, im.rangesB, nullptr);
+                       reinterpret_cast<float*>(b.grad_inst), b.inst_flag, g.touched, order, im.rangesB, nullptr, fill);
   }
   return hipGetLastError();
 }
diff --git a/include/gsraster.h b/include/gsraster.h
--- a/include/gsraster.h
+++ b/include/gsraster.h
@@ -49,6 +49,8 @@
 int gsr_async_outcomes_pending(void);
 unsigned long long gsr_async_outcomes_lost(void);
 unsigned long long gsr_frame_note_misses(void);
+int gsr_set_backward_fill(int on);
+unsigned long long gsr_backward_fills(void);
 unsigned gsr_near_budget_scale(void);
 unsigned gsr_near_budget_feedback(unsigned unfinished_quads, unsigned near_instances, unsigned far_instances);
 int gsr_near_far_pause(int frames);
```

New measurement: 1169 Mpixels/s. About the same (-0.4%).
